# rampasek/DrVAE

Hardware: AMD Instinct MI355X
Metric: DrVAE ELBO training samples/sec (batch x L) (higher is better)
Workload: dtype f32; 1 GPU; cfg2: DrVAE bortezomib shape: 978 genes, z1=z3=100, enc-z1 800, dec-x 600, enc-z3/dec-z1 200, batch 150/GPU, L=2; global_batch=150, L=2, parallelism=dp1, launch=hipGraph replay, feed=resident, side_chain_cus=64, rccl_ranks=0, params=2321758

## Files before the change

drvae_amd/_lib.py:

```python
import ctypes as C
import os

_HERE = os.path.dirname(os.path.abspath(__file__))
LIB_PATH = os.path.join(_HERE, 'libdrvae_hip.so')

ACT = {'identity': 0, 'elu': 1, 'softplus': 2, 'sigmoid': 3, 'tanh': 4, 'relu': 5, 'leaky_relu': 6, 'selu': 7,
       'softsign': 8, 'cos': 9}
GAUSS_LOGVAR, GAUSS_SIGMA = 0, 1
REC_KIND = {'binary': 0, 'poisson': 1}
EPI_PLAIN, EPI_FWD, EPI_BWD, EPI_KLQ = 0, 1, 2, 3

_f, _i32, _i64, _u64, _p = C.c_float, C.c_int32, C.c_int64, C.c_uint64, C.c_void_p


class GemmDesc(C.Structure):
    _fields_ = [('M', _i32), ('N', _i32), ('K', _i32), ('a_kcontig', _i32), ('b_kcontig', _i32),
                ('A', _p), ('lda', _i64), ('A2', _p), ('lda2', _i64), ('K1', _i32), ('a_kscale', _p),
                ('B', _p), ('ldb', _i64), ('C', _p), ('ldc', _i64), ('alpha', _f), ('beta', _f),
                ('epilogue', _i32), ('scale', _p), ('bias', _p), ('split', _i32), ('act0', _i32), ('act1', _i32),
                ('shift0', _f), ('shift1', _f), ('resid', _p), ('ldr', _i64), ('resid_cols', _i32),
                ('yref', _p), ('ldy', _i64), ('a_colsum', _p), ('colsum_beta', _f), ('flags', _i32),
                ('pub_flag', _p), ('pub_ctr', _p), ('pub_add', _i32), ('tune', _p)]


# ... 98 lines not shown
                ('n_entries', _i32), ('max_rows', _i32), ('S', _i32), ('B', _i32), ('grp_ptr', _p), ('rows', _p), ('src', _p),
                ('cls', _p), ('W', _p), ('b', _p), ('a', _f), ('c', _f), ('w', _f), ('fac', _f), ('theta', _p), ('diff', _p),
                ('cnt', _p), ('m2', _p), ('value', _p), ('dz', _p), ('ldd', _i64)]


class LossTerm(C.Structure):
    _fields_ = [('x', _p), ('w', _p), ('n', _i32), ('scale', _f), ('out', _i32), ('row_len', _i32)]


SIGNATURES = {
    'dv_abi_version': [],
    'dv_error_string': [_i32],
    'dv_source_hash': [],
    'dv_gemm': [C.POINTER(GemmDesc), _p],
    'dv_gemm_pair': [C.POINTER(GemmDesc), C.POINTER(GemmDesc), _p],
    'dv_gemm_heads': [C.POINTER(GemmDesc), C.POINTER(HeadsEpi), _p],
    'dv_gemm_heads_tiles': [_i32],
    'dv_bn_fwd': [_p, _i64, _i32, _i32, _p, _p, _f, _p, _p, _p, _i64, _p, _p, _f, _i32, _p],
    'dv_bn_bwd': [_p, _i64, _p, _i64, _p, _p, _p, _i32, _i32, _p, _i64, _p, _p, _i32, _p],
    'dv_mask_scale': [_p, _i64, _p, _i64, _f, _i32, _i32, _p, _i64, _p],
    'dv_gemm_has_tiling': [_i32],
    'dv_colsum': [_p, _i64, _i32, _i32, _p, _f, _p],
    'dv_act_bwd': [_p, _i64, _p, _i64, _i32, _i32, _i32, _i32, _i32, _f, _f, _p],
    'dv_wn_scale': [_p, _i64, _p, _i32, _i32, _p, _p, _p],
    'dv_wn_bwd': [_p, _i64, _p, _i64, _p, _p, _i32, _i32, _p, _i64, _p, _f, _p],
    'dv_reparam_fwd': [_p, _p, _i64, _p, _i32, _i32, _i32, _p, _i64, _i32, _p, _i64, _p, _i64, _p, _i64, _p, _i64, _p,
                       _p],
    'dv_reparam_bwd_seg': [_p, _i64, _p, _i64, _p, _i64, _p, _p, _i32, _i32, _i32, _p, _i64, _p, _p, _p, _p, _i64, _f,
                           C.POINTER(Bump), C.POINTER(SegAdd), C.POINTER(Wait), C.POINTER(PriorKl), _p],
    'dv_z2f_post_bwd': [C.POINTER(Z2F), C.POINTER(Wait), _p],
    'dv_reparam_bwd': [_p, _i64, _p, _i64, _p, _i64, _p, _i32, _i32, _i32, _i32, _p, _p, _i64, _f, _p],
    'dv_kl_rows_fwd': [C.POINTER(KlRows), C.POINTER(Wait), _p],
    'dv_kl_rows_fwd_pair': [C.POINTER(KlRows), C.POINTER(KlRows), _p],
    'dv_kl_rows_bwd': [C.POINTER(KlRows), C.POINTER(KlRowsGrad), _p],
    'dv_gauss_nll_rows_fwd': [_p, _i64, _p, _p, _p, _i64, _i32, _i32, _i32, _p, _p, _p, _f, _p],
    'dv_gauss_nll_rows_fwdbwd': [_p, _p, _i64, _p, _p, _p, _i64, _i32, _i32, _i32, _i32, _f, _p, _p, _p, _i64, _p, _p, _p],
    'dv_gauss_nll_rows_raw_cs': [C.POINTER(NllRawCs), _p],
    'dv_nll_raw_cs_chunks': [_i32],
    'dv_nll_raw_cs_row_blocks': [_i32],
    'dv_rec_nll_rows': [_i32, _f, _p, _p, _i64, _p, _p, _i64, _i32, _i32, _p, _p, _i64, _p],
    'dv_gauss_nll_rows_bwd': [_p, _p, _i64, _p, _p, _p, _i64, _i32, _i32, _i32, _i32, _f, _p, _p, _i64, _p, _i64,
                              _f, _p],
    'dv_softmax_clamp_fwd': [_p, _i64, _i32, _i32, _i32, _p, _i64, _p],
    'dv_softmax_clamp_bwd': [_p, _i64, _p, _i64, _i32, _i32, _i32, _p, _i64, _f, _p],
    'dv_cat_terms_fwd': [_p, _i64, _i32, _i32, _p, _p, _i64, _p, _p, _i64, _p, _p, _p],
    'dv_cat_terms_bwd': [_p, _i64, _i32, _i32, _p, _p, _i64, _p, _p, _i64, _p, _p, _i64, _f, _p],
    'dv_smalln_linear_fwd': [_p, _i64, _i32, _p, _i64, _i32, _p, _i64, _p, _i32, _i32, _p, _i64, _p, _i64,
                             C.POINTER(Ymarg), _p, _p, _p],
    'dv_smalln_linear_bwd_data': [_p, _i64, _p, _i64, _p, _i64, _i32, _i32, _i32, C.POINTER(_p), C.POINTER(_i64),
                                  C.POINTER(_i32), C.POINTER(_i32), C.POINTER(_f), C.POINTER(_f), C.POINTER(_i32),
                                  C.POINTER(_f), _p, _i64, _p, _p],
    'dv_smalln_linear_bwd_weight': [_p, _i64, _p, _i64, _p, _i64, _i32, _p, _i64, _i32, _i32, _i32, _p, _i64, _p, _f,
                                    _p, _p, _i32, _p],
    'dv_ymarg_fwd': [_p, _i64, _p, _p, _p, _f, _p, _i32, _i32, _p, _p, _p],
    'dv_ymarg_fwdbwd': [_p, _i64, _p, _p, _p, _f, _p, _p, _p, _i32, _i32, _p, _p, _p, _p, _i64, _p],
    'dv_ymarg_bwd': [_p, _i64, _p, _p, _p, _f, _p, _p, _p, _i32, _i32, _p, _p, _i64, _p],
    'dv_ycont_fwd': [_p, _i64, _p, _p, _p, _i64, _f, _i32, _i32, _i32, _i32, _p, _p, _i64, _p, _i64, _p],
    'dv_ycont_bwd': [_p, _i64, _p, _p, _f, _i32, _p, _p, _p, _i64, _p, _i64, _i32, _i32, _i32, _p, _i64, _p, _p],
    'dv_mmd_rff_fwd': [_p, _i64, _i32, _p, _i64, _i32, _i32, _f, _p, _p, _p],
    'dv_mmd_rff_bwd': [_p, _i64, _i32, _i32, _p, _p, _f, _p, _i64, _p],
    'dv_nuisance_feed': [_p, _p, _i32, _p, _p, _i32, _p, _i32, _i32, _i32, _p, _i64, _p, _i64, _p, _p],
    'dv_mmd_grouped_fwd': [C.POINTER(MmdGrouped), _p],
    'dv_mmd_grouped_bwd': [C.POINTER(MmdGrouped), _p],
    'dv_rows_gather': [_p, _i64, _p, _i32, _i32, _p, _i64, _f, _p, _i32, _p, _i64, C.POINTER(Wait), _p],
    'dv_batch_feed': [C.POINTER(BatchFeed), C.POINTER(BatchMasks), C.POINTER(Wait), _p],
    'dv_batch_masks': [C.POINTER(BatchMasks), _p, _i32, _p, _p, _i32, _i32, _p],
    'dv_rows_segment_sum': [_p, _i64, _p, _p, _p, _i32, _i32, _p, _p, _i64, _f, C.POINTER(Wait), _p],
    'dv_weighted_sum': [_p, _p, _p, _i32, _f, _p, _f, _p],
    'dv_recon_row_stats': [_p, _i64, _p, _i64, _i32, _i32, _p, _p],
    'dv_recon_rows': [C.POINTER(ReconRows), _p],
    'dv_col_moments': [_p, _i64, _p, _i64, _i32, _i32, _p, _i32, _p, _p, _p],
    'dv_mmd_mix_fwd': [_p, _i64, _i32, _i32, _i32, _p, _i32, _p, _i64, _p, _i64, _p, _p],
    'dv_mmd_mix_bwd': [_p, _i64, _i32, _i32, _i32, _p, _i32, _p, _i64, _p, _i64, _p, _f, _p, _i64, _p, _p],
    'dv_mmd_mix_combine': [_p, _i32, _f, _p, _i32, _f, _p, _i32, _f, _p, _p],
    'dv_mmd_identity_fwd': [_p, _i64, _i32, _p, _i64, _i32, _i32, _p, _p, _p],
    'dv_mmd_identity_bwd': [_p, _p, _f, _i32, _i32, _p, _i64, _p],
    'dv_recon_finalize': [_p, _p, _i32, _i32, _p, _i32, _p, _p, _p],
    'dv_rank_metrics': [_p, _i64, _p, _p, _p, _i32, _i32, _i32, _i32, _p, _p, _p],
    'dv_loss_assemble': [C.POINTER(LossTerm), _i32, _p, _p, _p, _p, _i32, _p, _p],
    'dv_loss_assemble_after': [C.POINTER(Wait), C.POINTER(LossTerm), _i32, _p, _p, _p, C.POINTER(Bump), _p, _i32, _p, _p],
    'dv_axpby': [_p, _f, _p, _f, _i64, _p],
    'dv_adam_l2': [_p, _p, _p, _p, _i64, C.POINTER(AdamHyper), _p, _p, _i32, _p],
    'dv_adam_l2_gated': [_p, _p, _p, _p, _i64, C.POINTER(AdamHyper), _p, C.POINTER(Wait), _i64, _i64, _p, _i32, _p],
    'dv_adamax_l2': [_p, _p, _p, _p, _i64, C.POINTER(AdamHyper), _p, _p, _i32, _p],
    'dv_flag_publish': [_p, _p, _i32, _p],
    'dv_flag_wait': [_p, _p, _i32, _p, _i32, C.POINTER(Publish), _p],
    'dv_counter_add': [_p, _i32, _i64, _p],
    'dv_counters_add2': [_p, _i32, _i64, _p, _i32, _i64, _p, _p],
    'dv_fill_normal': [_p, _i64, _u64, _p, _p],
    'dv_fill_normal_rows': [_p, _p, _i32, _u64, _p, _p, _p],
}

_lib = None
ABI_VERSION = 12


def load():
    global _lib
    if _lib is not None:
        return _lib
    import torch
    path = os.environ.get('DRVAE_HIP_LIB', LIB_PATH)
    if not os.path.exists(path):
        raise RuntimeError(
            'drvae_amd: %s is missing -- build it with `python -m drvae_amd.build` (hipcc, gfx950). '
            'There is no CPU/PyTorch fallback for the hot path.' % LIB_PATH)
    lib = C.CDLL(path)
    for name, argtypes in SIGNATURES.items():
        try:
            fn = getattr(lib, name)
        except AttributeError as e:
            raise RuntimeError('drvae_amd: symbol %s missing from %s (stale build?)' % (name, LIB_PATH)) from e
        fn.argtypes = argtypes
        fn.restype = C.c_char_p if name in ('dv_error_string', 'dv_source_hash') else C.c_int
    if lib.dv_abi_version() != ABI_VERSION:
        raise RuntimeError('drvae_amd: ABI version mismatch in %s' % LIB_PATH)
    _lib = lib
    return lib


def check(code, what):
    if code != 0:
        msg = load().dv_error_string(code)
        raise RuntimeError('drvae_amd: %s failed: %s (%d)' % (what, msg.decode() if msg else '?', code))
```

drvae_amd/chain.py:

```python
import torch

from . import kernels as K


def _pad4(n):
    return (n + 3) // 4 * 4


def _whole_rows(t):
    b = t._base
    return (b is not None and b.dim() == 2 and t.dim() == 2 and b.is_contiguous() and t.stride() == (b.shape[1], 1)
            and b.shape[1] == _pad4(t.shape[1]) and (t.storage_offset() - b.storage_offset()) % b.shape[1] == 0)


class _Lin:

    def __init__(self, arena, wname, bname, gname=None, second=None, act='identity', act1=None, shift0=0.0,
                 shift1=0.0):
        if second is None:
            self.W, self.dW = arena.p(wname), arena.g(wname)
            self.b, self.db = arena.p(bname), arena.g(bname)
            self.g = arena.p(gname) if gname else None
            self.dg = arena.g(gname) if gname else None
            self.split = self.W.shape[0]
        else:
            w2, b2, g2 = second
            self.W, self.dW = arena.fused(arena.param, wname, w2), arena.fused(arena.grad, wname, w2)
            self.b, self.db = arena.fused(arena.param, bname, b2), arena.fused(arena.grad, bname, b2)
            self.g = arena.fused(arena.param, gname, g2) if gname and g2 else None
            self.dg = arena.fused(arena.grad, gname, g2) if gname and g2 else None
            self.split = arena.shapes[wname][0]
        self.N, self.Kin = self.W.shape
        self.act0, self.act1 = act, (act if act1 is None else act1)
        self.shift0, self.shift1 = shift0, shift1
        dev = self.W.device
        if self.g is not None:
            self.scale = torch.empty(self.N, device=dev)
            self.norm = torch.empty(self.N, device=dev)
            self.raw = torch.empty(self.N, self.Kin, device=dev)
        else:
            self.scale = self.norm = self.raw = None


class _Chain:

    def __init__(self, layers, M, device, resid_cols=0):
        self.layers, self.M, self.resid_cols = layers, M, resid_cols
        self.out = [torch.zeros(M, _pad4(l.N), device=device)[:, :l.N] for l in layers]
        self.dpre = [torch.zeros(M, _pad4(l.N), device=device)[:, :l.N] for l in layers[:-1]]

    @staticmethod
    def _pad_ok(t):
        if t.dim() != 2 or t.shape[1] % 4 == 0:
            return True
        ld = t.stride(0) if t.shape[0] > 1 else max(t.stride(0), t.shape[1])
        return ld == t.shape[1] or _whole_rows(t)

    def raw_last_ok(self):
        l = self.layers[-1]
        return l.g is None and l.split * 2 == l.N and l.act0 == 'identity' and self.resid_cols == 0

    def forward(self, inputs, resid=None, publish=None, heads=None, raw_last=False):
        x = list(inputs)
        for li, l in enumerate(self.layers):
            if l.g is not None:
                K.wn_scale(l.scale, l.norm, l.W, l.g)
            last = li == len(self.layers) - 1
            kpad = len(x) == 1 and self._pad_ok(x[0])
            if last and heads is not None:
                assert l.split * 2 == l.N
                K.linear_heads(heads.get('out', self.out[li]), x[0], l.W, l.b, split=l.split,
                               x2=x[1] if len(x) > 1 else None, scale=l.scale, act0=l.act0, act1=l.act1,
                               shift0=l.shift0, shift1=l.shift1, resid=resid,
                               resid_cols=self.resid_cols if resid is not None else 0, overread=True,
                               publish=publish if (li == 0 and l.g is None) else None,
                               sample=heads.get('sample'), nll=heads.get('nll'), kpad=kpad)
                return self.out[-1]
            if last and raw_last:
                assert self.raw_last_ok() and resid is None
                K.gemm(self.out[li], x[0], l.W, True, True, A2=x[1] if len(x) > 1 else None, overread=True,
                       publish=publish if li == 0 else None, kpad=kpad)
                return self.out[-1]
            K.linear_fwd(self.out[li], x[0], l.W, l.b, x2=x[1] if len(x) > 1 else None, scale=l.scale, split=l.split,
                         act0=l.act0, act1=l.act1, shift0=l.shift0, shift1=l.shift1,
                         resid=resid if last else None, resid_cols=self.resid_cols if (last and resid is not None) else 0,
                         overread=True, publish=publish if (li == 0 and l.g is None) else None, kpad=kpad)
            x = [self.out[li]]
        return self.out[-1]

    def backward(self, dpre_last, inputs, dinputs=None, publish_after_last=None, publish_first=None, db_last_done=False,
                 klq=None):
        dpre = dpre_last
        pending_pub = publish_first
        took_klq = False
        n_layers = len(self.layers)
        for li in range(n_layers - 1, -1, -1):
            l = self.layers[li]
            db = None if (db_last_done and li == n_layers - 1) else l.db
            srcs = list(inputs) if li == 0 else [self.out[li - 1]]
            if li == len(self.layers) - 2 and publish_after_last is not None:
                pending_pub = publish_after_last

            single_dst = li > 0 or (dinputs is not None and len(srcs) == 1 and dinputs[0] is not None
                                    and len(dinputs[0]) == 1)
            if l.g is None and len(srcs) == 1 and single_dst:
                if li > 0:
                    prev = self.layers[li - 1]
                    K.linear_bwd_pair(l.dW, db, self.dpre[li - 1], dpre, srcs[0], l.W, yref=self.out[li - 1],
                                      act=prev.act0, shift=prev.shift0, overread=True, publish=pending_pub,
                                      npad=self._pad_ok(srcs[0]), npad_x=True)
                    dpre = self.dpre[li - 1]
                else:
                    dst, alpha, beta = dinputs[0][0]
                    if klq is not None and beta == 0.0:
                        K.linear_bwd_pair(l.dW, db, None, dpre, srcs[0], l.W, alpha=alpha, overread=True, publish=pending_pub,
                                          npad=self._pad_ok(srcs[0]), klq=klq)
                        took_klq = True
                    else:
                        K.linear_bwd_pair(l.dW, db, dst, dpre, srcs[0], l.W, alpha=alpha, beta_x=beta, overread=True,
                                          publish=pending_pub, npad=self._pad_ok(srcs[0]), npad_x=_whole_rows(dst))
                pending_pub = None
                continue
            if pending_pub is not None:
                K.flag_publish(*pending_pub)
                pending_pub = None
            dW = l.raw if l.g is not None else l.dW
            c0 = 0
            for si, s in enumerate(srcs):
                w = s.shape[1]
                K.linear_bwd_weight(dW[:, c0:c0 + w], dpre, s, dbias=db if si == 0 else None, overread=True,
                                    npad=len(srcs) == 1 and l.g is None and self._pad_ok(s))
                c0 += w
            if l.g is not None:
                K.wn_bwd(l.dW, l.dg, l.raw, l.W, l.g, l.norm)
            if li > 0:
                prev = self.layers[li - 1]
                K.linear_bwd_data(self.dpre[li - 1], dpre, l.W, kscale=l.scale, yref=self.out[li - 1], act=prev.act0,
                                  shift=prev.shift0, overread=True, npad=True)
                dpre = self.dpre[li - 1]
            elif dinputs is not None:
                c0 = 0
                for si, s in enumerate(srcs):
                    w = s.shape[1]
                    for (dst, alpha, beta) in (dinputs[si] or []):
                        K.linear_bwd_data(dst, dpre, l.W[:, c0:c0 + w], kscale=l.scale, alpha=alpha, beta=beta,
                                          overread=True)
                    c0 += w
        return took_klq
```

drvae_amd/csrc/gemm.hip:

```cpp
#include "gemm_common.inc"

namespace {

#include "gemm_pipe.inc"


struct Operand {
    const float* base;
    int64_t ld;
    int n_line, n_pos;
};

__device__ __forceinline__ float4 ld_fast(const Operand& o, int line, int pos, int vec) {
    const float* p = o.base + (int64_t)line * o.ld + pos;
    if (vec == 4) return *reinterpret_cast<const float4*>(p);
    if (vec == 2) {
        const float2 a = *reinterpret_cast<const float2*>(p), b = *reinterpret_cast<const float2*>(p + 2);
        return make_float4(a.x, a.y, b.x, b.y);
    }
    return make_float4(p[0], p[1], p[2], p[3]);
}

__device__ __forceinline__ float4 ld_edge(const Operand& o, int line, int pos) {
    const bool lok = line < o.n_line;
    const float* row = o.base + (int64_t)(lok ? line : o.n_line - 1) * o.ld;
    float e[4];
#pragma unroll
    for (int j = 0; j < 4; ++j) {
        const int q = pos + j;
        const float v = row[q < o.n_pos ? q : o.n_pos - 1];
        e[j] = (lok && q < o.n_pos) ? v : 0.f;
    }
    return make_float4(e[0], e[1], e[2], e[3]);
}

template <int BM, int RPT>
__device__ __forceinline__ int heads_row0(int grp) { return (grp & 1) * (BM / 2) + (grp >> 1) * RPT; }

template <int BM, int BN, int KS, int NT>
__device__ __forceinline__ void heads_epilogue(const dv_gemm_desc& g, const dv_heads_epi& he, const float* red, int m0,
                                               int tn, int tiles_n, int pre_s0, int pre_s1) {
    constexpr int HB = BN / 2, RPT = BM / (NT / HB);
    constexpr bool PRE = (KS == 8 && BN == 32);
    static_assert(!PRE || RPT == 1, "prefetched bounds: one row per thread");
    static_assert((HB == 32 || HB == 16) && RPT >= 1, "half tile = 16 or 32 adjacent lanes");
    static_assert((NT / HB) % 2 == 0 && (BM / 2) % RPT == 0, "row groups come in pairs");
    const int tid = threadIdx.x, c = tid % HB, r0 = heads_row0<BM, RPT>(tid / HB);
    const int col0 = tn * HB + c, col1 = g.split + col0;
    const bool ok = col0 < g.split && col1 < g.N;
    const int cc0 = ok ? col0 : g.split - 1, cc1 = ok ? col1 : g.N - 1;
    float sc0 = 1.f, sc1 = 1.f, bi0 = 0.f, bi1 = 0.f;
    if (g.scale) {
        sc0 = g.scale[cc0];
        sc1 = g.scale[cc1];
    }
    if (g.bias) {
        bi0 = g.bias[cc0];
        bi1 = g.bias[cc1];
    }
    const bool use_res = g.resid != nullptr && col0 < g.resid_cols;
#pragma unroll
    for (int e = 0; e < RPT; ++e) {
        const int row = m0 + r0 + e;
        const bool rok = row < g.M;
        const int rc = rok ? row : g.M - 1;
        float v0 = 0.f, v1 = 0.f;
#pragma unroll
        for (int w = 0; w < KS; ++w) {
            v0 += red[(w * BM + r0 + e) * (BN + 1) + c];
            v1 += red[(w * BM + r0 + e) * (BN + 1) + HB + c];
        }
        float a0 = dv_act(g.act0, v0 * g.alpha * sc0 + bi0) + g.shift0;
        if (use_res) a0 += g.resid[(int64_t)rc * g.ldr + cc0];
        if (he.mode == DV_HEADS_NLL && g.act1 == DV_ACT_SOFTPLUS) {
            const float pre = v1 * g.alpha * sc1 + bi1;
            const float e_ = __expf(-fabsf(pre));
            const float r1 = __frcp_rn(1.f + e_);
            const float sd = fmaxf(pre, 0.f) + dv_log1p_hw(e_, r1) + g.shift1;
            const float sig = (pre >= 0.f ? 1.f : e_) * r1;
            const float is = __frcp_rn(sd);
            const float xv = he.x[(int64_t)(he.xidx ? he.xidx[rc] : rc) * he.ldx + cc0];
            const float cf = he.coef[rc];
            const float t = (xv - a0) * is;
            float acc = ok ? kLog2PiG + 2.f * __logf(sd) + t * t : 0.f;
            if (ok && rok) {
                g.C[(int64_t)row * g.ldc + col0] = cf * t * is;
                g.C[(int64_t)row * g.ldc + col1] = cf * (t * t - 1.f) * is * sig;
            }
#pragma unroll
            for (int off = HB / 2; off > 0; off >>= 1) acc += __shfl_xor(acc, off, 64);
            if (c == 0 && rok) he.part[(int64_t)row * tiles_n + tn] = -0.5f * acc;
            continue;
        }
        const float a1 = dv_act(g.act1, v1 * g.alpha * sc1 + bi1) + g.shift1;
        if (he.mode == DV_HEADS_SAMPLE) {
            if (ok && rok) {
                g.C[(int64_t)row * g.ldc + col0] = a0;
                g.C[(int64_t)row * g.ldc + col1] = a1;
                if (row < he.n_src) {
                    const float std_ = expf(0.5f * a1);
                    const int s0 = he.seg_ptr ? (PRE ? pre_s0 : he.seg_ptr[row]) : row;
                    const int s1 = he.seg_ptr ? (PRE ? pre_s1 : he.seg_ptr[row + 1]) : row + 1;
                    for (int t = s0; t < s1; ++t) {
                        const int64_t s = he.seg_rows ? he.seg_rows[t] : t;
                        const float z = he.eps[s * he.lde + col0] * std_ + a0;
                        he.out[s * he.ldo + col0] = z;
                        if (he.out2) he.out2[s * he.ldo2 + col0] = z - he.sub[s * he.lds + col0];
                        if (he.out3) {
                            const int t3 = he.out3_idx[s];
                            if (t3 >= 0) he.out3[(int64_t)t3 * he.ldo3 + col0] = z;
                        }
                        if (he.out4)
                            for (int u = he.out4_ptr[s]; u < he.out4_ptr[s + 1]; ++u) he.out4[(int64_t)u * he.ldo4 + col0] = z;
                    }
                }
            }
        } else {
            const float xv = he.x[(int64_t)(he.xidx ? he.xidx[rc] : rc) * he.ldx + cc0];
            const float cf = he.coef[rc];
            const float d = xv - a0, v = a1 * a1;
            float acc = ok ? kLog2PiG + logf(v) + d * d / v : 0.f;
            float gm = d / v, gs = -1.f / a1 + d * d / (v * a1);
            if (g.act1 != DV_ACT_IDENTITY) gs *= dv_dact_from_y(g.act1, a1 - g.shift1);
            gm *= cf;
            gs *= cf;
            if (ok && rok) {
                g.C[(int64_t)row * g.ldc + col0] = gm;
                g.C[(int64_t)row * g.ldc + col1] = gs;
            }
#pragma unroll
            for (int off = HB / 2; off > 0; off >>= 1) acc += __shfl_xor(acc, off, 64);
            if (c == 0 && rok) he.part[(int64_t)row * tiles_n + tn] = -0.5f * acc;
        }
    }
}

template <int BM, int BN, int BK, int KS, bool AKC, bool BKC, int PS = 0>
constexpr int gemm_smem_floats() {
    if constexpr (PS > 0) return PipeGeom<BM, BN, BK, BM / 32, BN / 32, KS, PS, AKC, BKC>::SMEM_FL;
    constexpr int stage = (AKC ? BM : BK) * ((AKC ? BK : BM) + 4) + (BKC ? BN : BK) * ((BKC ? BK : BN) + 4);
    constexpr int red = (KS > 1) ? KS * BM * (BN + 1) : 0;
    return 2 * stage > red ? 2 * stage : red;
}

template <int BM, int BN, int BK, int WM, int WN, int KS, bool AKC, bool BKC, bool PAIR = false, bool MI16 = false, int PS = 0>
__device__ __forceinline__ void gemm_body(const dv_gemm_desc& g, const LoadCfg& lc, float* smem, int bid, int nwg,
                                          const dv_heads_epi* he = nullptr) {
    static_assert(!PAIR || (AKC && BKC && KS > 1 && WM == 1 && WN == 1), "paired heads: forward layout, K-split tiling");
    constexpr int HB = BN / 2;
    static_assert(!MI16 || (KS == 1 && !PAIR), "16x16x4 tiles: unsplit K only");
    constexpr int TS = MI16 ? 16 : 32;
    constexpr int AR = MI16 ? 4 : 16;
    constexpr int TM = BM / WM / TS, TN = BN / WN / TS;
    constexpr int KW = BK / KS, KH = KW / (MI16 ? 4 : 2);
    constexpr int LDA_S = (AKC ? BK : BM) + 4;
    constexpr int LDB_S = (BKC ? BK : BN) + 4;
    constexpr int A_ELEMS = (AKC ? BM : BK) * LDA_S;
    constexpr int B_ELEMS = (BKC ? BN : BK) * LDB_S;
    constexpr int STAGE = A_ELEMS + B_ELEMS;
    constexpr int RED_ELEMS = (KS > 1) ? KS * BM * (BN + 1) : 0;
    constexpr int NT = 64 * WM * WN * KS;
    static_assert(PS > 0 || (2 * STAGE <= gemm_smem_floats<BM, BN, BK, KS, AKC, BKC>() && RED_ELEMS <= gemm_smem_floats<BM, BN, BK, KS, AKC, BKC>()), "smem");
    static_assert(PS == 0 || (!MI16 && TM == 1 && TN == 1), "pipe loop inside gemm_body: one 32x32 tile per wave");
    static_assert(NT == 256 || NT == 512 || NT == 1024, "4, 8 or 16 waves");

    const bool ones_col = BM < 128 && !AKC && !BKC && (g.flags & DV_FLAG_ONES_COL);
    const int tiles_m = (g.M + BM - 1) / BM;
    const int tiles_n = PAIR ? (g.split + HB - 1) / HB : (g.N + (ones_col ? DV_ONES_OFF(g) + 1 : 0) + BN - 1) / BN;
    int tm, tn;
    tile_of_block(bid, nwg, tiles_m, tiles_n, lc.map, tm, tn);
    const int m0 = tm * BM, n0 = tn * BN;
    auto bline = [&](int l) -> int {
        if (PAIR) {
            const int c = tn * HB + (l < HB ? l : l - HB);
            return l < HB ? (c < g.split ? c : g.split - 1) : (g.split + c < g.N ? g.split + c : g.N - 1);
        }
        return n0 + l < g.N ? n0 + l : g.N - 1;
    };

    const int tid = threadIdx.x, lane = tid & 63, wave = tid >> 6;
    const int li = MI16 ? (lane & 15) : (lane & 31), lh = MI16 ? (lane >> 4) : (lane >> 5);
    const int ks_id = wave / (WM * WN);
    const int wm = (wave % (WM * WN)) / WN, wn = wave % WN;

    constexpr int A_CPL = (AKC ? BK : BM) / 4;
    constexpr int A_LPP = NT / A_CPL;
    constexpr int A_NP = (AKC ? BM : BK) / A_LPP;
    constexpr int B_CPL = (BKC ? BK : BN) / 4;
    constexpr int B_LPP = NT / B_CPL;
    constexpr int B_NP = (BKC ? BN : BK) / B_LPP;
    static_assert(A_NP >= 1 && B_NP >= 1, "tile too small for the workgroup");
    const int a_c = tid % A_CPL, a_l = tid / A_CPL;
    const int b_c = tid % B_CPL, b_l = tid / B_CPL;
    const int oc = (ones_col && n0 <= g.N && g.N < n0 + BN) ? g.N - n0 - b_c * 4 : -1;

    const Operand oa{g.A, g.lda, AKC ? g.M : g.K, AKC ? g.K : g.M};
    const Operand ob{g.B, g.ldb, BKC ? g.N : g.K, BKC ? g.K : g.N};
    const bool a_plain = g.A2 == nullptr;
    const bool a_int = AKC ? true : (m0 + BM <= g.M);
    const bool b_int = BKC ? true : (n0 + BN <= g.N);
    const bool wg_fast = a_plain && (a_int || (g.flags & 1)) && (b_int || (g.flags & 2)) && g.a_kscale == nullptr;

    auto gen_load = [&](int k0, float4 (&ra)[A_NP], float4 (&rb)[B_NP]) {
#pragma unroll
        for (int p = 0; p < A_NP; ++p) {
            const int l = a_l + p * A_LPP;
            const int line = AKC ? (m0 + l) : (k0 + l);
            const int pos = AKC ? (k0 + a_c * 4) : (m0 + a_c * 4);
            float4 v;
            if (a_plain) {
                v = ld_edge(oa, line, pos);
            } else {
                const bool lok = line < g.M;
                const int64_t r = lok ? line : g.M - 1;
                float e[4];
#pragma unroll
                for (int j = 0; j < 4; ++j) {
                    const int q = pos + j, qc = q < g.K ? q : g.K - 1;
                    const float* src = qc >= g.K1 ? g.A2 + r * g.lda2 + (qc - g.K1) : g.A + r * g.lda + qc;
                    const float x = *src;
                    e[j] = (lok && q < g.K) ? x : 0.f;
                }
                v = make_float4(e[0], e[1], e[2], e[3]);
            }
            if (AKC && g.a_kscale) {
                const int kq = g.K - 1;
                v.x *= g.a_kscale[pos < kq ? pos : kq];
                v.y *= g.a_kscale[pos + 1 < kq ? pos + 1 : kq];
                v.z *= g.a_kscale[pos + 2 < kq ? pos + 2 : kq];
                v.w *= g.a_kscale[pos + 3 < kq ? pos + 3 : kq];
// ... 26 lines not shown
        }
    };

    typename std::conditional<MI16, f32x4, f32x16>::type acc[TM][TN];
#pragma unroll
    for (int i = 0; i < TM; ++i)
#pragma unroll
        for (int j = 0; j < TN; ++j)
#pragma unroll
            for (int r = 0; r < AR; ++r) acc[i][j][r] = 0.f;

    int pre_s0 = 0, pre_s1 = 0;
    if constexpr (PAIR && KS == 8 && BN == 32) {
        if (he->mode == DV_HEADS_SAMPLE && he->seg_ptr != nullptr) {
            const int prow = m0 + heads_row0<BM, 1>(tid / (BN / 2));
            if (prow < he->n_src && prow < g.M) {
                pre_s0 = he->seg_ptr[prow];
                pre_s1 = he->seg_ptr[prow + 1];
            }
        }
    }
    const int kb = ks_id * KW + lh * KH;
    auto read_frags = [&](const float* sA, float (&fa)[TM][KH], float (&fb)[TN][KH]) {
        const float* sB = sA + A_ELEMS;
#pragma unroll
        for (int i = 0; i < TM; ++i) {
            const int row = wm * TM * TS + i * TS + li;
#pragma unroll
            for (int s = 0; s < KH; s += 4) {
                if (AKC) {
                    const float4 v = *reinterpret_cast<const float4*>(&sA[row * LDA_S + kb + s]);
                    fa[i][s] = v.x;
                    fa[i][s + 1] = v.y;
                    fa[i][s + 2] = v.z;
                    fa[i][s + 3] = v.w;
                } else {
#pragma unroll
                    for (int e = 0; e < 4; ++e) fa[i][s + e] = sA[(kb + s + e) * LDA_S + row];
                }
            }
        }
#pragma unroll
        for (int j = 0; j < TN; ++j) {
            const int col = wn * TN * TS + j * TS + li;
#pragma unroll
            for (int s = 0; s < KH; s += 4) {
                if (BKC) {
                    const float4 v = *reinterpret_cast<const float4*>(&sB[col * LDB_S + kb + s]);
                    fb[j][s] = v.x;
                    fb[j][s + 1] = v.y;
                    fb[j][s + 2] = v.z;
                    fb[j][s + 3] = v.w;
                } else {
#pragma unroll
                    for (int e = 0; e < 4; ++e) fb[j][s + e] = sB[(kb + s + e) * LDB_S + col];
                }
            }
        }
    };
    auto mma = [&](const float (&fa)[TM][KH], const float (&fb)[TN][KH]) {
#pragma unroll
        for (int s = 0; s < KH; ++s)
#pragma unroll
            for (int i = 0; i < TM; ++i)
#pragma unroll
                for (int j = 0; j < TN; ++j) {
                    if constexpr (MI16)
                        acc[i][j] = __builtin_amdgcn_mfma_f32_16x16x4f32(fa[i][s], fb[j][s], acc[i][j], 0, 0, 0);
                    else if (DV_DBG & 2)
                        acc[i][j][s & 15] += fa[i][s] * fb[j][s];
                    else
                        acc[i][j] = __builtin_amdgcn_mfma_f32_32x32x2f32(fa[i][s], fb[j][s], acc[i][j], 0, 0, 0);
                }
    };
    auto compute = [&](const float* sA) {
        float fa[TM][KH], fb[TN][KH];
        read_frags(sA, fa, fb);
        mma(fa, fb);
    };

    const int nkt = (g.K + BK - 1) / BK, nfull = g.K / BK;
    float* const buf0 = smem;
    float* const buf1 = smem + STAGE;
    if constexpr (PS > 0) {
        if (!(DV_DBG & 64))
            pipe_loop<BM, BN, BK, WM, WN, KS, PS, AKC, BKC, (BM < 128 && !AKC && !BKC)>(
                g, smem, m0, n0, [&](int l) { return m0 + l < g.M ? m0 + l : g.M - 1; }, bline, acc);
        if (DV_DBG & 128) {
            if (acc[0][0][0] == 12345.678f) g.C[0] = acc[0][0][1];
            return;
        }
        __syncthreads();
    } else if (wg_fast && nfull >= 1) {
        const float* pa[A_NP];
        const float* pb[B_NP];
#pragma unroll
        for (int p = 0; p < A_NP; ++p) {
            const int l = a_l + p * A_LPP;
            int line = AKC ? (m0 + l) : l;
            if (AKC) line = line < g.M ? line : g.M - 1;
            pa[p] = g.A + (int64_t)line * g.lda + (AKC ? a_c * 4 : (m0 + a_c * 4 < g.M ? m0 + a_c * 4 : 0));
        }
#pragma unroll
        for (int p = 0; p < B_NP; ++p) {
            const int l = b_l + p * B_LPP;
            const int line = BKC ? bline(l) : l;
            pb[p] = g.B + (int64_t)line * g.ldb + (BKC ? b_c * 4 : (n0 + b_c * 4 < g.N ? n0 + b_c * 4 : 0));
        }
        const int64_t step_a = AKC ? (int64_t)BK : (int64_t)BK * g.lda;
        const int64_t step_b = BKC ? (int64_t)BK : (int64_t)BK * g.ldb;
        const int va = lc.vecA, vb = lc.vecB;
        auto ldv = [](const float* p, int vec) -> float4 {
            if (vec == 4) return *reinterpret_cast<const float4*>(p);
            if (vec == 2) {
                const float2 a = *reinterpret_cast<const float2*>(p), b = *reinterpret_cast<const float2*>(p + 2);
                return make_float4(a.x, a.y, b.x, b.y);
            }
            return make_float4(p[0], p[1], p[2], p[3]);
        };
        auto ldv_tail = [](const float* p, int vec, int left) -> float4 {
            const float* z = dv_zero_chunk;
            if (vec == 4) return *reinterpret_cast<const float4*>(left >= 4 ? p : z);
            if (vec == 2) {
                const float2 a = *reinterpret_cast<const float2*>(left >= 2 ? p : z);
                const float2 b = *reinterpret_cast<const float2*>(left >= 4 ? p + 2 : z);
                return make_float4(a.x, a.y, b.x, b.y);
            }
            return make_float4(*(left >= 1 ? p : z), *(left >= 2 ? p + 1 : z), *(left >= 3 ? p + 2 : z),
                               *(left >= 4 ? p + 3 : z));
        };
        auto fetch = [&](int t, float4 (&ra)[A_NP], float4 (&rb)[B_NP]) {
            if (t < nfull) {
#pragma unroll
                for (int p = 0; p < A_NP; ++p) {
                    ra[p] = ldv(pa[p], va);
                    pa[p] += step_a;
                }
#pragma unroll
                for (int p = 0; p < B_NP; ++p) {
                    rb[p] = ldv(pb[p], vb);
                    pb[p] += step_b;
                }
            } else {
                const int kt0 = nfull * BK;
#pragma unroll
                for (int p = 0; p < A_NP; ++p) {
                    if (AKC) {
                        ra[p] = ldv_tail(pa[p], lc.vecA_t, g.K - (kt0 + a_c * 4));
                    } else {
                        ra[p] = ldv((kt0 + a_l + p * A_LPP < g.K) ? pa[p] : dv_zero_chunk, va);
                    }
                }
#pragma unroll
                for (int p = 0; p < B_NP; ++p) {
                    if (BKC) {
                        rb[p] = ldv_tail(pb[p], lc.vecB_t, g.K - (kt0 + b_c * 4));
                    } else {
                        rb[p] = ldv((kt0 + b_l + p * B_LPP < g.K) ? pb[p] : dv_zero_chunk, vb);
                    }
                }
            }
        };
        float4 a0[A_NP], b0[B_NP], a1[A_NP], b1[B_NP];
#if DV_STAMP
        const bool stamp_on = dv_stamp_buf != nullptr && wave == 0;
        int si = 2;
#endif
// ... 49 lines not shown
            }
            if (!(DV_DBG & 8)) __syncthreads();
            if (kt + 1 >= nkt) break;
            compute(buf1);
            if (kt + 2 < nkt) {
                if (!(DV_DBG & 4)) stage_store(buf0, a0, b0);
                if (kt + 4 < nkt && !(DV_DBG & 1)) fetch(kt + 4, a0, b0);
            }
            if (!(DV_DBG & 8)) __syncthreads();
        }
    } else {
        float4 ra[A_NP], rb[B_NP];
        gen_load(0, ra, rb);
        stage_store(buf0, ra, rb);
        __syncthreads();
        for (int kt = 0; kt < nkt; ++kt) {
            if (kt + 1 < nkt) gen_load((kt + 1) * BK, ra, rb);
            compute((kt & 1) ? buf1 : buf0);
            if (kt + 1 < nkt) stage_store((kt & 1) ? buf0 : buf1, ra, rb);
            __syncthreads();
        }
    }

    if constexpr (MI16) {
#pragma unroll
        for (int i = 0; i < TM; ++i)
#pragma unroll
            for (int j = 0; j < TN; ++j) {
                float a4[4];
#pragma unroll
                for (int r = 0; r < 4; ++r) a4[r] = acc[i][j][r];
                const int rbase = m0 + wm * TM * TS + i * TS + 4 * lh;
                epi_store_col<4, (BM < 128)>(g, a4, n0 + wn * TN * TS + j * TS + li, [rbase](int r) { return rbase + r; });
            }
    } else if constexpr (KS == 1) {
#pragma unroll
        for (int i = 0; i < TM; ++i)
#pragma unroll
            for (int j = 0; j < TN; ++j) {
                float a16[16];
#pragma unroll
                for (int r = 0; r < 16; ++r) a16[r] = acc[i][j][r];
                const int rbase = m0 + wm * TM * 32 + i * 32 + 4 * lh;
                epi_store_col<16, (BM < 128)>(g, a16, n0 + wn * TN * 32 + j * 32 + li,
                                  [rbase](int r) { return rbase + (r & 3) + 8 * (r >> 2); });
            }
    } else {
        float* red = smem;
        if constexpr (PAIR) {
#pragma unroll
            for (int j = 0; j < TN; ++j)
#pragma unroll
                for (int r = 0; r < 16; ++r) {
                    const int row = (r & 3) + 8 * (r >> 2) + 4 * lh;
                    red[(ks_id * BM + row) * (BN + 1) + j * 32 + li] = acc[0][j][r];
                }
            __syncthreads();
            heads_epilogue<BM, BN, KS, NT>(g, *he, red, m0, tn, tiles_n, pre_s0, pre_s1);
            return;
        }
#pragma unroll
        for (int i = 0; i < TM; ++i)
#pragma unroll
            for (int j = 0; j < TN; ++j)
#pragma unroll
                for (int r = 0; r < 16; ++r) {
                    const int row = wm * TM * 32 + i * 32 + (r & 3) + 8 * (r >> 2) + 4 * lh;
                    const int col = wn * TN * 32 + j * 32 + li;
                    red[(ks_id * BM + row) * (BN + 1) + col] = acc[i][j][r];
                }
        __syncthreads();
        constexpr int RPT = BM / (NT / BN);
        const int col = tid % BN, r0 = (tid / BN) * RPT;
        float a4[RPT];
#pragma unroll
        for (int e = 0; e < RPT; ++e) {
            float v = 0.f;
#pragma unroll
            for (int w = 0; w < KS; ++w) v += red[(w * BM + r0 + e) * (BN + 1) + col];
            a4[e] = v;
        }
        const int rbase = m0 + r0;
        epi_store_col<RPT>(g, a4, n0 + col, [rbase](int r) { return rbase + r; });
    }
}


template <int BM, int BN, int BK, int WM, int WN, int KS, bool AKC, bool BKC, bool MI16 = false>
__global__ __launch_bounds__(64 * WM * WN * KS, (WM * WN * KS == 16) ? 4 : (BM >= 128 || BK >= 128) ? 2 : (BM * BN >= 6144) ? (WM * WN * KS) / 4 : (WM * WN * KS == 8 ? (BM * BN == 1024 ? DV_LB8 : 2) : (BK == 32 && BM == 32 ? ((AKC || BKC) ? DV_DENSE_WG : DV_DENSE_WG - 1) : 4))) void gemm_kernel(const dv_gemm_desc g, const LoadCfg lc) {
    __shared__ __attribute__((aligned(16))) float smem[gemm_smem_floats<BM, BN, BK, KS, AKC, BKC>()];
    publish_on_entry(g);
#if DV_STAGGER
    {
        const int ph = (blockIdx.x / DV_STAGGER) & 3;
        if (ph == 1) __builtin_amdgcn_s_sleep(6);
        if (ph == 2) __builtin_amdgcn_s_sleep(12);
        if (ph == 3) __builtin_amdgcn_s_sleep(18);
    }
#endif
    gemm_body<BM, BN, BK, WM, WN, KS, AKC, BKC, false, MI16>(g, lc, smem, blockIdx.x, gridDim.x);
}

#ifdef DV_LAB
template <int KS, int NBUF = 3>
__global__ __launch_bounds__(64 * KS, NBUF > 4 ? KS / 4 : (KS == 8 ? 2 : 4)) void gemm_dma_kernel(const dv_gemm_desc g, const LoadCfg lc) {
    constexpr int BM = 32, BN = 32, BK = 64, NT = 64 * KS, KW = BK / KS, KH = KW / 2;
    constexpr int TILE = 32 * BK, STAGE = 2 * TILE, RED = KS * BM * (BN + 1);
    constexpr int PIECES = 16 / KS;
    static_assert((NBUF - 2) * PIECES <= 63, "vmcnt is a 6-bit counter");
    __shared__ __attribute__((aligned(16))) float smem[NBUF * STAGE > RED ? NBUF * STAGE : RED];
    publish_on_entry(g);
    const int tiles_m = (g.M + BM - 1) / BM, tiles_n = (g.N + BN - 1) / BN;
    int tm, tn;
    tile_of_block(blockIdx.x, gridDim.x, tiles_m, tiles_n, lc.map, tm, tn);
    const int m0 = tm * BM, n0 = tn * BN;
    const int tid = threadIdx.x, lane = tid & 63, wave = tid >> 6;
    const int li = lane & 31, lh = lane >> 5;

    const float* src[PIECES];
    int kofs[PIECES];
    int dst[PIECES];
#pragma unroll
    for (int i = 0; i < PIECES; ++i) {
        const int q = wave + i * KS, o = q >> 3, row = 4 * (q & 7) + (lane >> 4), p = lane & 15;
        const int c = p ^ (row & 15);
        int line = (o == 0 ? m0 : n0) + row;
        const int lim = o == 0 ? g.M : g.N;
        line = line < lim ? line : lim - 1;
        src[i] = (o == 0 ? g.A + (int64_t)line * g.lda : g.B + (int64_t)line * g.ldb) + c * 4;
        kofs[i] = c * 4;
        dst[i] = o * TILE + (q & 7) * 256;
    }
    auto issue = [&](int kt, float* stage) {
#pragma unroll
        for (int i = 0; i < PIECES; ++i) {
            const float* p = (kt * BK + kofs[i] < g.K) ? src[i] + (int64_t)kt * BK : dv_zero_chunk;
            __builtin_amdgcn_global_load_lds(p, (__attribute__((address_space(3))) float*)(stage + dst[i]), 16, 0, 0);
        }
    };
    f32x16 acc;
#pragma unroll
    for (int r = 0; r < 16; ++r) acc[r] = 0.f;
    const int kb = wave * KW + lh * KH;
    const int nkt = (g.K + BK - 1) / BK;
#pragma unroll
    for (int t = 0; t < NBUF - 1; ++t) issue(t, smem + t * STAGE);
    int bi = 0;
    for (int kt = 0; kt < nkt; ++kt) {
        float* cur = smem + bi * STAGE;
        asm volatile("s_waitcnt vmcnt(%0)" ::"n"((NBUF - 2) * PIECES) : "memory");
        asm volatile("s_barrier" ::: "memory");
        int bn = bi + NBUF - 1;
        bn = bn >= NBUF ? bn - NBUF : bn;
        issue(kt + NBUF - 1, smem + bn * STAGE);
        bi = bi + 1 == NBUF ? 0 : bi + 1;
        float fa[KH], fb[KH];
#pragma unroll
        for (int s = 0; s < KH; s += 4) {
            const int pc = (((kb + s) >> 2) ^ (li & 15)) << 2;
            const float4 va = *reinterpret_cast<const float4*>(&cur[li * BK + pc]);
            const float4 vb = *reinterpret_cast<const float4*>(&cur[TILE + li * BK + pc]);
            fa[s] = va.x; fa[s + 1] = va.y; fa[s + 2] = va.z; fa[s + 3] = va.w;
            fb[s] = vb.x; fb[s + 1] = vb.y; fb[s + 2] = vb.z; fb[s + 3] = vb.w;
        }
#pragma unroll
        for (int s = 0; s < KH; ++s) acc = __builtin_amdgcn_mfma_f32_32x32x2f32(fa[s], fb[s], acc, 0, 0, 0);
// ... 70 lines not shown
        const float4 x0 = *reinterpret_cast<const float4*>(&(ST)[li * LD + lh * 8]);       \
        const float4 x1 = *reinterpret_cast<const float4*>(&(ST)[li * LD + lh * 8 + 4]);   \
        const float4 y0 = *reinterpret_cast<const float4*>(&(ST)[OPER + li * LD + lh * 8]);     \
        const float4 y1 = *reinterpret_cast<const float4*>(&(ST)[OPER + li * LD + lh * 8 + 4]); \
        acc = __builtin_amdgcn_mfma_f32_32x32x2f32(x0.x, y0.x, acc, 0, 0, 0);              \
        acc = __builtin_amdgcn_mfma_f32_32x32x2f32(x0.y, y0.y, acc, 0, 0, 0);              \
        acc = __builtin_amdgcn_mfma_f32_32x32x2f32(x0.z, y0.z, acc, 0, 0, 0);              \
        acc = __builtin_amdgcn_mfma_f32_32x32x2f32(x0.w, y0.w, acc, 0, 0, 0);              \
        acc = __builtin_amdgcn_mfma_f32_32x32x2f32(x1.x, y1.x, acc, 0, 0, 0);              \
        acc = __builtin_amdgcn_mfma_f32_32x32x2f32(x1.y, y1.y, acc, 0, 0, 0);              \
        acc = __builtin_amdgcn_mfma_f32_32x32x2f32(x1.z, y1.z, acc, 0, 0, 0);              \
        acc = __builtin_amdgcn_mfma_f32_32x32x2f32(x1.w, y1.w, acc, 0, 0, 0);              \
    }
    if (s0 < s1) {
        float* st0 = my;
        float* st1 = my + STAGE;
        WP_FETCH(s0, a00, a01, b00, b01);
        WP_FETCH(s0 + 1, a10, a11, b10, b11);
        WP_STASH(st0, a00, a01, b00, b01);
        WP_FETCH(s0 + 2, a00, a01, b00, b01);
        const int n = s1 - s0;
        int s = s0;
        for (int it = 0; it < n / 2; ++it, s += 2) {
            WP_STASH(st1, a10, a11, b10, b11);
            WP_FETCH(s + 3, a10, a11, b10, b11);
            WP_MMA(st0);
            WP_STASH(st0, a00, a01, b00, b01);
            WP_FETCH(s + 4, a00, a01, b00, b01);
            WP_MMA(st1);
        }
        if (n & 1) WP_MMA(st0);
    }
#undef WP_FETCH
#undef WP_STASH
#undef WP_MMA
    __syncthreads();
    float* red = smem;
#pragma unroll
    for (int r = 0; r < 16; ++r) red[(wave * BM + (r & 3) + 8 * (r >> 2) + 4 * lh) * (BN + 1) + li] = acc[r];
    __syncthreads();
    constexpr int RPT = BM / (256 / BN);
    const int col = tid % BN, r0 = (tid / BN) * RPT;
    float a4[RPT];
#pragma unroll
    for (int e = 0; e < RPT; ++e) {
        float v = 0.f;
#pragma unroll
        for (int w = 0; w < KS; ++w) v += red[(w * BM + r0 + e) * (BN + 1) + col];
        a4[e] = v;
    }
    const int rbase = m0 + r0;
    epi_store_col<RPT>(g, a4, n0 + col, [rbase](int r) { return rbase + r; });
}

#endif

template <int BM, int BN, int BK, int KS>
__global__ __launch_bounds__(64 * KS, KS == 8 ? 2 : (BK == 32 ? DV_DENSE_WG : 4)) void gemm_heads_kernel(const dv_gemm_desc g, const LoadCfg lc,
                                                               const dv_heads_epi he) {
    __shared__ __attribute__((aligned(16))) float smem[gemm_smem_floats<BM, BN, BK, KS, true, true>()];
    publish_on_entry(g);
    gemm_body<BM, BN, BK, 1, 1, KS, true, true, true>(g, lc, smem, blockIdx.x, gridDim.x, &he);
}

template <int BM, int BN, int BK, int WM, int WN, int KS, bool A1, bool B1, bool A2, bool B2>
__global__ __launch_bounds__(256, BK == 32 ? DV_DENSE_WG : 4) void gemm_pair_kernel(const dv_gemm_desc g1, const LoadCfg lc1, const dv_gemm_desc g2,
                                                        const LoadCfg lc2, int tiles1) {
    constexpr int S1 = gemm_smem_floats<BM, BN, BK, KS, A1, B1>(), S2 = gemm_smem_floats<BM, BN, BK, KS, A2, B2>();
    __shared__ __attribute__((aligned(16))) float smem[S1 > S2 ? S1 : S2];
    publish_on_entry(g1);
    if ((int)blockIdx.x < tiles1)
        gemm_body<BM, BN, BK, WM, WN, KS, A1, B1>(g1, lc1, smem, blockIdx.x, tiles1);
    else
        gemm_body<BM, BN, BK, WM, WN, KS, A2, B2>(g2, lc2, smem, blockIdx.x - tiles1, gridDim.x - tiles1);
}

template <int BM, int BN, int BK, int KS, bool AKC, bool BKC, int PS, int WPS>
__global__ __launch_bounds__(64 * KS * (BM / 32) * (BN / 32), WPS) void gemm_kpipe_kernel(const dv_gemm_desc g, const LoadCfg lc) {
    __shared__ __attribute__((aligned(1024))) float smem[gemm_smem_floats<BM, BN, BK, KS, AKC, BKC, PS>()];
    publish_on_entry(g);
    gemm_body<BM, BN, BK, BM / 32, BN / 32, KS, AKC, BKC, false, false, PS>(g, lc, smem, blockIdx.x, gridDim.x);
}

template <int BM, int BN, int BK, int KS, int PS, int WPS>
__global__ __launch_bounds__(64 * KS, WPS) void gemm_heads_pipe_kernel(const dv_gemm_desc g, const LoadCfg lc, const dv_heads_epi he) {
    __shared__ __attribute__((aligned(1024))) float smem[gemm_smem_floats<BM, BN, BK, KS, true, true, PS>()];
    publish_on_entry(g);
    gemm_body<BM, BN, BK, 1, 1, KS, true, true, true, false, PS>(g, lc, smem, blockIdx.x, gridDim.x, &he);
}

template <int BM, int BN, int BK, int KS, bool A1, bool B1, bool A2, bool B2, int PS, int WPS>
__global__ __launch_bounds__(256, WPS) void gemm_pair_pipe_kernel(const dv_gemm_desc g1, const LoadCfg lc1, const dv_gemm_desc g2,
                                                                    const LoadCfg lc2, int tiles1) {
    constexpr int S1 = gemm_smem_floats<BM, BN, BK, KS, A1, B1, PS>(), S2 = gemm_smem_floats<BM, BN, BK, KS, A2, B2, PS>();
    __shared__ __attribute__((aligned(1024))) float smem[S1 > S2 ? S1 : S2];
    publish_on_entry(g1);
    if ((int)blockIdx.x < tiles1)
        gemm_body<BM, BN, BK, 1, 1, KS, A1, B1, false, false, PS>(g1, lc1, smem, blockIdx.x, tiles1);
    else
        gemm_body<BM, BN, BK, 1, 1, KS, A2, B2, false, false, PS>(g2, lc2, smem, blockIdx.x - tiles1, gridDim.x - tiles1);
}

inline int vec_width(const void* p, int64_t ld) {
    const uintptr_t a = reinterpret_cast<uintptr_t>(p);
    if ((a & 15) == 0 && (ld & 3) == 0) return 4;
    if ((a & 7) == 0 && (ld & 1) == 0) return 2;
    return 1;
}

const dv_gemm_tune k_default_tune = {0, {-1, 0, 0, 0, 0, 0, 0, 0, 0, 0}};
inline const dv_gemm_tune& tune_of(const dv_gemm_desc& g) { return g.tune != nullptr ? *g.tune : k_default_tune; }
inline int lds_pad(const dv_gemm_desc& g, int bm, int tiles) { return (bm <= 32 && tiles >= 512) ? tune_of(g).opt[1] : 0; }

inline int cols_eff(const dv_gemm_desc& g) { return g.N + ((g.flags & DV_FLAG_ONES_COL) ? DV_ONES_OFF(g) + 1 : 0); }

template <int BM, int BN, int BK, int WM, int WN, int KS, bool MI16 = false>
int launch_cfg(const dv_gemm_desc& g, const LoadCfg& lc, hipStream_t st) {
    const int tiles = ((g.M + BM - 1) / BM) * ((cols_eff(g) + BN - 1) / BN);
    dim3 grid(tiles), block(64 * WM * WN * KS);
    if (g.a_kcontig && g.b_kcontig)
        hipLaunchKernelGGL((gemm_kernel<BM, BN, BK, WM, WN, KS, true, true, MI16>), grid, block, lds_pad(g, BM, tiles), st, g, lc);
    else if (g.a_kcontig && !g.b_kcontig)
        hipLaunchKernelGGL((gemm_kernel<BM, BN, BK, WM, WN, KS, true, false, MI16>), grid, block, lds_pad(g, BM, tiles), st, g, lc);
    else if (!g.a_kcontig && !g.b_kcontig)
        hipLaunchKernelGGL((gemm_kernel<BM, BN, BK, WM, WN, KS, false, false, MI16>), grid, block, lds_pad(g, BM, tiles), st, g, lc);
    else
        return DV_ERR_UNSUPPORTED;
    DV_RETURN_LAUNCH();
}

inline void pipe_ones_off(dv_gemm_desc& g) {
    if (g.flags & DV_FLAG_ONES_COL) g.flags = (g.flags & ~0x300) | (((4 - (g.N & 3)) & 3) << 8);
}

template <int BM, int BN, int BK, int KS, int PS, int WPS>
int launch_kpipe(const dv_gemm_desc& g_in, const LoadCfg& lc, hipStream_t st) {
    dv_gemm_desc g = g_in;
    pipe_ones_off(g);
    const int tiles = ((g.M + BM - 1) / BM) * ((cols_eff(g) + BN - 1) / BN);
    dim3 grid(tiles), block(64 * KS * (BM / 32) * (BN / 32));
    if (g.a_kcontig && g.b_kcontig)
        hipLaunchKernelGGL((gemm_kpipe_kernel<BM, BN, BK, KS, true, true, PS, WPS>), grid, block, 0, st, g, lc);
    else if (g.a_kcontig && !g.b_kcontig)
        hipLaunchKernelGGL((gemm_kpipe_kernel<BM, BN, BK, KS, true, false, PS, WPS>), grid, block, 0, st, g, lc);
    else if (!g.a_kcontig && !g.b_kcontig)
        hipLaunchKernelGGL((gemm_kpipe_kernel<BM, BN, BK, KS, false, false, PS, WPS>), grid, block, 0, st, g, lc);
    else
        return DV_ERR_UNSUPPORTED;
    DV_RETURN_LAUNCH();
}

}

extern "C" int dv_gemm_has_tiling(int t) {
#ifndef DV_LAB
    return ((t >= 0 && t <= 3) || t == 17 || t == 40 || t == 46) ? 1 : 0;
#else
    return t >= 0 ? 1 : 0;
#endif
}

#if DV_STAMP
extern "C" int dv_gemm_stamp_buffer(unsigned long long* p) {
    return hipMemcpyToSymbol(HIP_SYMBOL(dv_stamp_buf), &p, sizeof(p)) == hipSuccess ? DV_OK : DV_ERR_LAUNCH;
}
#endif
// ... 114 lines not shown
            DV_RETURN_LAUNCH();
        }
        return launch_cfg<32, 32, 64, 1, 1, 8>(g, lc, st);
    }
    if (tiling == 11 || tiling == 12 || (tiling >= 21 && tiling <= 24)) {
        const bool ok = g.a_kcontig && g.b_kcontig && g.A2 == nullptr && g.a_kscale == nullptr && (g.K & 3) == 0 &&
                        lc.vecA == 4 && lc.vecB == 4;
        if (ok) {
            const int tiles = ((g.M + 31) / 32) * ((g.N + 31) / 32);
            if (tiling == 11)
                hipLaunchKernelGGL((gemm_dma_kernel<8>), dim3(tiles), dim3(512), 0, st, g, lc);
            else if (tiling == 12)
                hipLaunchKernelGGL((gemm_dma_kernel<4>), dim3(tiles), dim3(256), 0, st, g, lc);
            else if (tiling == 21)
                hipLaunchKernelGGL((gemm_dma_kernel<8, 5>), dim3(tiles), dim3(512), 0, st, g, lc);
            else if (tiling == 22)
                hipLaunchKernelGGL((gemm_dma_kernel<8, 9>), dim3(tiles), dim3(512), 0, st, g, lc);
            else if (tiling == 23)
                hipLaunchKernelGGL((gemm_dma_kernel<4, 5>), dim3(tiles), dim3(256), 0, st, g, lc);
            else
                hipLaunchKernelGGL((gemm_dma_kernel<4, 9>), dim3(tiles), dim3(256), 0, st, g, lc);
            DV_RETURN_LAUNCH();
        }
        return launch_cfg<32, 32, 64, 1, 1, 8>(g, lc, st);
    }
#endif
    if (tiling == 17) return launch_cfg<32, 32, 32, 1, 1, 4>(g, lc, st);
    if (tiling != 1 && tiling != 2) return DV_ERR_UNSUPPORTED;
    if (tiling == 1) return launch_cfg<64, 64, 32, 2, 2, 1>(g, lc, st);
    const int tiles32 = ((g.M + 31) / 32) * ((cols_eff(g) + 31) / 32);
    const bool pipe = pipe_on(g) && pipe_ok(g, lc);
    if (tiles32 >= dense_min_tiles(g)) return pipe ? launch_kpipe<32, 32, 32, 4, 2, DV_DENSE_WG>(g, lc, st) : launch_cfg<32, 32, 32, 1, 1, 4>(g, lc, st);
    if (g.a_kcontig && tune_of(g).opt[7] == 0) return pipe ? launch_kpipe<32, 32, 64, 8, 2, 2>(g, lc, st) : launch_cfg<32, 32, 64, 1, 1, 8>(g, lc, st);
    return pipe ? launch_kpipe<32, 32, 64, 4, 2, 4>(g, lc, st) : launch_cfg<32, 32, 64, 1, 1, 4>(g, lc, st);
}

static bool ragged_n_split_pays(const dv_gemm_desc& g, int tiling) {
    if (tiling != 40 || tune_of(g).tiling != 0 || tune_of(g).opt[6] == -1) return false;
    const int n_tail = g.N % 256, n_main = g.N - n_tail;
    if (n_tail == 0 || n_main == 0) return false;
    const int64_t rows_t = (g.M + 127) / 128, kCUs = 256;
    const int64_t full = rows_t * ((g.N + 255) / 256), main = rows_t * (n_main / 256);
    return (full + kCUs - 1) / kCUs > (main + kCUs - 1) / kCUs;
}

extern "C" int dv_gemm(const dv_gemm_desc* d, dv_stream_t stream) {
    LoadCfg lc;
    int tiling = 0;
    const int rc = gemm_prepare(d, lc, tiling);
    if (rc != DV_OK) return rc;
    if (ragged_n_split_pays(*d, tiling)) {
        const int n_tail = d->N % 256, n_main = d->N - n_tail;
        dv_gemm_desc g1 = *d, g2 = *d;
        g1.N = n_main;
        g2.N = n_tail;
        g2.B = d->B + (d->b_kcontig ? (int64_t)n_main * d->ldb : (int64_t)n_main);
        g2.C = d->C + n_main;
        g1.split = d->split < n_main ? d->split : n_main;
        g2.split = d->split > n_main ? d->split - n_main : 0;
        if (d->scale) g2.scale = d->scale + n_main;
        if (d->bias) g2.bias = d->bias + n_main;
        if (d->yref) g2.yref = d->yref + n_main;
        if (d->resid) {
            g1.resid_cols = d->resid_cols < n_main ? d->resid_cols : n_main;
            g2.resid_cols = d->resid_cols > n_main ? d->resid_cols - n_main : 0;
            g2.resid = g2.resid_cols > 0 ? d->resid + n_main : nullptr;
        }
        g2.a_colsum = nullptr;
        g2.pub_flag = nullptr;
        g2.tune = nullptr;
        LoadCfg l1, l2;
        int t1 = 0, t2 = 0;
        int r = gemm_prepare(&g1, l1, t1);
        if (r != DV_OK) return r;
        r = gemm_prepare(&g2, l2, t2);
        if (r != DV_OK) return r;
        r = gemm_launch(g1, l1, t1, static_cast<hipStream_t>(stream));
        if (r != DV_OK) return r;
        return gemm_launch(g2, l2, t2, static_cast<hipStream_t>(stream));
    }
    return gemm_launch(*d, lc, tiling, static_cast<hipStream_t>(stream));
}

#ifdef DV_LAB
static int heads_hb() { return 16; }
#else
static int heads_hb() { return 16; }
#endif
extern "C" int dv_gemm_heads_tiles(int32_t split) { return split > 0 ? (split + heads_hb() - 1) / heads_hb() : 0; }

extern "C" int dv_gemm_heads(const dv_gemm_desc* d, const dv_heads_epi* e, dv_stream_t stream) {
    LoadCfg lc;
    int tiling = 0;
    DV_REQUIRE(d != nullptr && e != nullptr);
    const int rc = gemm_prepare(d, lc, tiling);
    if (rc != DV_OK) return rc;
    if (tiling < 0) return DV_OK;
    const dv_gemm_desc& g = *d;
    DV_REQUIRE(g.a_kcontig && g.b_kcontig && g.epilogue == DV_EPI_FWD && g.beta == 0.f && g.a_colsum == nullptr);
    DV_REQUIRE(g.split > 0 && g.N == 2 * g.split && g.resid_cols <= g.split);
    DV_REQUIRE(e->mode == DV_HEADS_SAMPLE || e->mode == DV_HEADS_NLL);
    if (e->mode == DV_HEADS_SAMPLE) {
        DV_REQUIRE(e->eps && e->out && e->n_src >= 0 && e->n_src <= g.M);
        DV_REQUIRE((e->seg_ptr == nullptr) == (e->seg_rows == nullptr));
        DV_REQUIRE(e->out2 == nullptr || e->sub != nullptr);
        DV_REQUIRE(e->out3 == nullptr || e->out3_idx != nullptr);
        DV_REQUIRE(e->out4 == nullptr || e->out4_ptr != nullptr);
    } else {
        DV_REQUIRE(e->x && e->coef && e->part);
    }
    lc.map = tune_of(g).opt[0] >= 0 ? tune_of(g).opt[0] : 1;
    const int tiles = ((g.M + 31) / 32) * dv_gemm_heads_tiles(g.split);
#ifdef DV_LAB
    if (tune_of(g).opt[4] == 1) {
        hipLaunchKernelGGL((gemm_heads_kernel<32, 64, 64, 4>), dim3(tiles), dim3(256), 0,
                           static_cast<hipStream_t>(stream), g, lc, *e);
        DV_RETURN_LAUNCH();
    }
    if (tune_of(g).opt[4] == 2) {
        hipLaunchKernelGGL((gemm_heads_kernel<32, 64, 64, 8>), dim3(tiles), dim3(512), 0,
                           static_cast<hipStream_t>(stream), g, lc, *e);
        DV_RETURN_LAUNCH();
    }
    if (tune_of(g).opt[4] == -1) {
        hipLaunchKernelGGL((gemm_heads_kernel<32, 32, 64, 4>), dim3(tiles), dim3(256), 0,
                           static_cast<hipStream_t>(stream), g, lc, *e);
        DV_RETURN_LAUNCH();
    }
#endif
    const bool pipe = pipe_on(g) && pipe_ok(g, lc);
    if (tune_of(g).opt[4] == 3 || (tune_of(g).opt[4] == 0 && tiles >= dense_min_tiles(g))) {
        if (pipe)
            hipLaunchKernelGGL((gemm_heads_pipe_kernel<32, 32, 32, 4, 2, DV_DENSE_WG>), dim3(tiles), dim3(256), 0,
                               static_cast<hipStream_t>(stream), g, lc, *e);
        else
            hipLaunchKernelGGL((gemm_heads_kernel<32, 32, 32, 4>), dim3(tiles), dim3(256), 0,
                               static_cast<hipStream_t>(stream), g, lc, *e);
    } else if (pipe) {
        hipLaunchKernelGGL((gemm_heads_pipe_kernel<32, 32, 64, 8, 2, 2>), dim3(tiles), dim3(512), 0,
                           static_cast<hipStream_t>(stream), g, lc, *e);
    } else {
        hipLaunchKernelGGL((gemm_heads_kernel<32, 32, 64, 8>), dim3(tiles), dim3(512), lds_pad(g, 32, tiles),
                           static_cast<hipStream_t>(stream), g, lc, *e);
    }
    DV_RETURN_LAUNCH();
}

extern "C" int dv_gemm_pair(const dv_gemm_desc* d1, const dv_gemm_desc* d2, dv_stream_t stream) {
    LoadCfg lc1, lc2;
    int t1 = 0, t2 = 0;
    int rc = gemm_prepare(d1, lc1, t1);
    if (rc != DV_OK) return rc;
    rc = gemm_prepare(d2, lc2, t2);
    if (rc != DV_OK) return rc;
    hipStream_t st = static_cast<hipStream_t>(stream);
    DV_REQUIRE(!(d1->pub_flag != nullptr && d2->pub_flag != nullptr));
    dv_gemm_desc e1 = *d1, e2 = *d2;
    e2.flags &= 3;
    if (t1 == 2 && t2 == 2) {
        rc = colsum_setup(e1, 2, st);
        if (rc != DV_OK) return rc;
    }
    const bool pipe = pipe_on(e1) && t1 == 2 && t2 == 2 && pipe_ok(e1, lc1) && pipe_ok(e2, lc2);
    if (pipe) pipe_ones_off(e1);
    const int tiles1 = ((e1.M + 31) / 32) * ((cols_eff(e1) + 31) / 32), tiles2 = ((e2.M + 31) / 32) * ((e2.N + 31) / 32);
    const bool fuse = t1 == 2 && t2 == 2 && !d1->a_kcontig && !d1->b_kcontig && d2->a_kcontig && !d2->b_kcontig &&
// ... 38 lines not shown
```

drvae_amd/csrc/gemm_pipe.inc:

```

template <int BM, int BN, int BK, int WM, int WN, int KS, int S, bool AKC, bool BKC>
struct PipeGeom {
    static constexpr int NW = WM * WN * KS, NT = 64 * NW;
    static constexpr int TM = BM / WM / 32, TN = BN / WN / 32;
    static constexpr int KW = BK / KS, KH = KW / 2, G = KH / 4;
    static constexpr int A_FL = BM * BK, B_FL = BN * BK, STAGE_FL = A_FL + B_FL;
    static constexpr int PA = A_FL / 256, PB = B_FL / 256, P = (PA + PB) / NW;
    static constexpr int CPR = BK / 4;
    static constexpr int RED_FL = (KS > 1) ? KS * BM * (BN + 1) : 0;
    static constexpr int SMEM_FL = S * STAGE_FL > RED_FL ? S * STAGE_FL : RED_FL;
    static_assert(KH % 4 == 0 && G >= 1, "a lane half holds whole 16-B chunks of k");
    static_assert((PA + PB) % NW == 0 && P >= 1, "pieces divide over the waves");
    static_assert(CPR == 4 || CPR == 8 || CPR == 16, "BK = 16, 32 or 64");
    static_assert(TM == 1 || TM == 2 || TM == 4, "row-contiguous reads are 4, 8 or 16 B");
    static_assert(TN == 1 || TN == 2 || TN == 4, "row-contiguous reads are 4, 8 or 16 B");
    static_assert(AKC || (256 % BM == 0 && BM <= 256), "row-contiguous A: whole k lines per piece");
    static_assert(BKC || (256 % BN == 0 && BN <= 256), "row-contiguous B: whole k lines per piece");
    static_assert((S - 2) * P <= 63 && S >= 2, "vmcnt is a 6-bit counter");
};

template <int CPR>
__device__ __forceinline__ int pipe_sw(int row) {
    return (row / (16 / CPR)) & (CPR - 1);
}

template <int N>
__device__ __forceinline__ void pipe_wait_vm() {
    asm volatile("s_waitcnt vmcnt(%0)" ::"n"(N) : "memory");
}

template <int BM, int BN, int BK, int WM, int WN, int KS, int S, bool AKC, bool BKC, bool ONES = false, typename LineA,
          typename LineB>
__device__ __forceinline__ void pipe_loop(const dv_gemm_desc& g, float* smem, int m0, int n0, LineA a_line,
                                          LineB b_line, f32x16 (&acc)[BM / WM / 32][BN / WN / 32]) {
    using PG = PipeGeom<BM, BN, BK, WM, WN, KS, S, AKC, BKC>;
    constexpr int TM = PG::TM, TN = PG::TN, G = PG::G, P = PG::P, CPR = PG::CPR, NW = PG::NW;
    const int tid = threadIdx.x, lane = tid & 63;
    const int wave = __builtin_amdgcn_readfirstlane(tid >> 6);
    const int li = lane & 31, lh = lane >> 5;
    const int ks_id = wave / (WM * WN), wm = (wave % (WM * WN)) / WN, wn = wave % WN;

    unsigned voff[P];
    int kofs[P];
    bool live[P];
    const bool ones_on = ONES && (g.flags & DV_FLAG_ONES_COL) != 0;
    const int n_ones = g.N + DV_ONES_OFF(g);
#pragma unroll
    for (int i = 0; i < P; ++i) {
        const int q = wave + i * NW;
        const bool isA = q < PG::PA;
        const int pq = isA ? q : q - PG::PA;
        const bool kc = isA ? AKC : BKC;
        const int64_t ld = isA ? g.lda : g.ldb;
        live[i] = true;
        if (kc) {
            const int row_t = pq * (64 / CPR) + lane / CPR;
            const int c = (lane % CPR) ^ pipe_sw<CPR>(row_t);
            const int T = isA ? TM : TN, wq = row_t / (T * 32), jq = (row_t / 32) % T, lq = row_t % 32;
            const int line = isA ? a_line(wq * T * 32 + T * lq + jq) : b_line(wq * T * 32 + T * lq + jq);
            kofs[i] = c * 4;
            voff[i] = (unsigned)(((int64_t)line * ld + c * 4) * 4);
        } else {
            const int R = isA ? BM : BN;
            const int line_t = pq * (256 / R) + lane / (R / 4), rc = lane % (R / 4);
            const int r0 = isA ? m0 : n0, lim = isA ? g.M : g.N;
            const int col = r0 + rc * 4 < lim ? r0 + rc * 4 : 0;
            kofs[i] = line_t;
            voff[i] = (unsigned)(((int64_t)line_t * ld + col) * 4);
            if (ONES && !isA) live[i] = !(ones_on && r0 + rc * 4 == n_ones);
        }
    }
    const int64_t step_a = (AKC ? (int64_t)BK : (int64_t)BK * g.lda) * 4, step_b = (BKC ? (int64_t)BK : (int64_t)BK * g.ldb) * 4;
    const char* base_a = reinterpret_cast<const char*>(g.A);
    const char* base_b = reinterpret_cast<const char*>(g.B);
    int k_issued = 0;
    const unsigned lds0 = (unsigned)(uintptr_t)smem;
    auto issue_piece = [&](auto full, int i, unsigned stage_byte) {
        const int q = wave + i * NW;
        const unsigned dst = __builtin_amdgcn_readfirstlane(lds0 + stage_byte + q * 1024);
        const char* base = q < PG::PA ? base_a : base_b;
        if (DV_DBG & 16) return;
        if constexpr (decltype(full)::value) {
            if (!ONES || live[i])
                asm volatile("s_mov_b32 m0, %1\n\ts_nop 0\n\tglobal_load_lds_dwordx4 %0, %2" ::"v"(voff[i]), "s"(dst), "s"(base) : "memory");
        } else if (!ONES || live[i]) {
            const char* p = kofs[i] < g.K - k_issued ? base + voff[i] : reinterpret_cast<const char*>(dv_zero_chunk);
            asm volatile("s_mov_b32 m0, %1\n\ts_nop 0\n\tglobal_load_lds_dwordx4 %0, off" ::"v"(p), "s"(dst) : "memory");
        }
    };
    auto issued = [&]() {
        base_a += step_a;
        base_b += step_b;
        k_issued += BK;
    };
    const int kb = ks_id * PG::KW + lh * PG::KH;
    const int swl = pipe_sw<CPR>(li);
    constexpr int NRA = AKC ? TM : 4, NRB = BKC ? TN : 4, NR = NRA + NRB;
    auto read_ops = [&](const float* stage, int gi, float (&fa)[TM][4], float (&fb)[TN][4], int lo, int hi) {
        const float* sA = stage;
        const float* sB = stage + PG::A_FL;
        const int c = ((kb >> 2) + gi) ^ swl;
#pragma unroll
        for (int r = 0; r < NRA; ++r) {
            if (r < lo || r >= hi) continue;
            if constexpr (AKC) {
                const float4 v = *reinterpret_cast<const float4*>(&sA[(wm * TM * 32 + r * 32 + li) * BK + c * 4]);
                fa[r][0] = v.x; fa[r][1] = v.y; fa[r][2] = v.z; fa[r][3] = v.w;
            } else {
                const float* p = &sA[(kb + gi * 4 + r) * BM + wm * TM * 32 + TM * li];
                if constexpr (TM == 4) {
                    const float4 v = *reinterpret_cast<const float4*>(p);
                    fa[0][r] = v.x; fa[1][r] = v.y; fa[2][r] = v.z; fa[3][r] = v.w;
                } else if constexpr (TM == 2) {
                    const float2 v = *reinterpret_cast<const float2*>(p);
                    fa[0][r] = v.x; fa[1][r] = v.y;
                } else {
                    fa[0][r] = *p;
                }
            }
        }
#pragma unroll
        for (int r = 0; r < NRB; ++r) {
            if (NRA + r < lo || NRA + r >= hi) continue;
            if constexpr (BKC) {
                const float4 v = *reinterpret_cast<const float4*>(&sB[(wn * TN * 32 + r * 32 + li) * BK + c * 4]);
                fb[r][0] = v.x; fb[r][1] = v.y; fb[r][2] = v.z; fb[r][3] = v.w;
            } else {
                const float* p = &sB[(kb + gi * 4 + r) * BN + wn * TN * 32 + TN * li];
                if constexpr (TN == 4) {
                    const float4 v = *reinterpret_cast<const float4*>(p);
                    fb[0][r] = v.x; fb[1][r] = v.y; fb[2][r] = v.z; fb[3][r] = v.w;
                } else if constexpr (TN == 2) {
                    const float2 v = *reinterpret_cast<const float2*>(p);
                    fb[0][r] = v.x; fb[1][r] = v.y;
                } else {
                    fb[0][r] = *p;
                }
            }
        }
    };
    auto read_group = [&](const float* stage, int gi, float (&fa)[TM][4], float (&fb)[TN][4]) {
        read_ops(stage, gi, fa, fb, 0, NR);
    };
    auto mma = [&](const float (&fa)[TM][4], const float (&fb)[TN][4], int lo, int hi) {
#pragma unroll
        for (int s = 0; s < 4; ++s)
#pragma unroll
            for (int i = 0; i < TM; ++i)
#pragma unroll
                for (int j = 0; j < TN; ++j) {
                    const int n = (s * TM + i) * TN + j;
                    if (n >= lo && n < hi) {
                        if (DV_DBG & 32) {
                            acc[i][j][0] += fa[i][s] + fb[j][s];
                        } else {
                            acc[i][j] = __builtin_amdgcn_mfma_f32_32x32x2f32(fa[i][s], fb[j][s], acc[i][j], 0, 0, 0);
                        }
                    }
                }
    };
    constexpr int NM = 4 * TM * TN;
    constexpr int RPM = (NR + NM - 1) / NM > 2 ? (NR + NM - 1) / NM : 2, NSL = (NR + RPM - 1) / RPM;
    static_assert(NSL <= NM, "reads dealt out over the group's MFMAs");
    const int nkt = (g.K + BK - 1) / BK;
    if constexpr (ONES) {
        if (ones_on && n0 <= n_ones && n_ones < n0 + BN && tid < S * BK)
            *reinterpret_cast<float4*>(&smem[(tid / BK) * PG::STAGE_FL + PG::A_FL + (tid % BK) * BN + (n_ones - n0)]) =
                make_float4(1.f, 1.f, 1.f, 1.f);
    }
#pragma unroll
    for (int t = 0; t < S; ++t) {
        if (k_issued + BK <= g.K) {
#pragma unroll
            for (int i = 0; i < P; ++i) issue_piece(std::true_type{}, i, t * PG::STAGE_FL * 4);
        } else {
#pragma unroll
            for (int i = 0; i < P; ++i) issue_piece(std::false_type{}, i, t * PG::STAGE_FL * 4);
        }
        issued();
    }
    asm volatile("s_waitcnt lgkmcnt(0)" ::: "memory");
    pipe_wait_vm<(S - 1) * P>();
    __builtin_amdgcn_s_barrier();
    float fa0[TM][4], fb0[TN][4], fa1[TM][4], fb1[TN][4];
    read_group(smem, 0, fa0, fb0);
    int sc = 0;
    auto tile = [&](auto full, float (&xa)[TM][4], float (&xb)[TN][4], float (&ya)[TM][4], float (&yb)[TN][4]) {
        const float* cur = smem + sc * PG::STAGE_FL;
        const int sn = sc + 1 == S ? 0 : sc + 1;
        const float* nxt = smem + sn * PG::STAGE_FL;
#pragma unroll
        for (int gi = 0; gi < G; ++gi) {
            float(&ca)[TM][4] = (gi & 1) ? ya : xa;
            float(&cb)[TN][4] = (gi & 1) ? yb : xb;
            float(&na)[TM][4] = (gi & 1) ? xa : ya;
            float(&nb)[TN][4] = (gi & 1) ? xb : yb;
            if (gi + 1 < G) {
                mma(ca, cb, 0, 1);
                __builtin_amdgcn_sched_barrier(0);
#pragma unroll
                for (int q = 0; q < NSL; ++q) {
                    read_ops(cur, gi + 1, na, nb, q * RPM, (q + 1) * RPM);
                    __builtin_amdgcn_sched_barrier(0);
                    if (q + 1 < NSL) {
                        mma(ca, cb, 1 + q, 2 + q);
                        __builtin_amdgcn_sched_barrier(0);
                    }
                }
                mma(ca, cb, NSL, NM);
                __builtin_amdgcn_sched_barrier(0);
            } else {
                asm volatile("s_waitcnt lgkmcnt(0)" ::: "memory");
                pipe_wait_vm<(S - 2) * P>();
                __builtin_amdgcn_s_barrier();
                asm volatile("" ::: "memory");
                mma(ca, cb, 0, 1);
                __builtin_amdgcn_sched_barrier(0);
#pragma unroll
                for (int q = 0; q < NSL; ++q) {
                    read_ops(nxt, 0, na, nb, q * RPM, (q + 1) * RPM);
                    __builtin_amdgcn_sched_barrier(0);
                    if (q + 1 < NSL) {
                        mma(ca, cb, 1 + q, 2 + q);
                        __builtin_amdgcn_sched_barrier(0);
                    }
                }
                const unsigned sb = sc * PG::STAGE_FL * 4;
                constexpr int M0 = NSL, ML = NM - M0;
#pragma unroll
                for (int i = 0; i < P; ++i) {
                    mma(ca, cb, M0 + i * ML / (P + 1), M0 + (i + 1) * ML / (P + 1));
                    __builtin_amdgcn_sched_barrier(0);
                    issue_piece(full, i, sb);
                    __builtin_amdgcn_sched_barrier(0);
                }
                mma(ca, cb, M0 + P * ML / (P + 1), NM);
                __builtin_amdgcn_sched_barrier(0);
                issued();
            }
        }
        sc = sn;
    };
    const int nfast = g.K / BK - S;
    int kt = 0;
    if constexpr (G % 2 == 0) {
        for (; kt < nfast; ++kt) tile(std::true_type{}, fa0, fb0, fa1, fb1);
        for (; kt < nkt; ++kt) tile(std::false_type{}, fa0, fb0, fa1, fb1);
    } else {
        for (; kt + 1 < nfast; kt += 2) {
            tile(std::true_type{}, fa0, fb0, fa1, fb1);
            tile(std::true_type{}, fa1, fb1, fa0, fb0);
        }
        for (; kt + 1 < nkt; kt += 2) {
            tile(std::false_type{}, fa0, fb0, fa1, fb1);
            tile(std::false_type{}, fa1, fb1, fa0, fb0);
        }
        if (kt < nkt) tile(std::false_type{}, fa0, fb0, fa1, fb1);
    }
    pipe_wait_vm<0>();
}

template <int BM, int BN, int WM, int WN, bool AKC, bool BKC>
__device__ __forceinline__ void pipe_epilogue(const dv_gemm_desc& g, int m0, int n0,
// ... 181 lines not shown
```

drvae_amd/csrc/optim.hip:

```cpp
#include "dv_common.h"
#include <cstring>

namespace {

struct AdamC {
    float lr_over_bc1, inv_unused, bc2_sqrt, eps, wd, one_minus_b1, b2, one_minus_b2, gscale;
};

__device__ __forceinline__ void adam_consts(float lr, float b1, float b2, const int32_t* step_dev, float* step_size,
                                            float* bc2_sqrt) {
    const double t = (double)step_dev[0];
    const double bc1 = 1.0 - pow((double)b1, t);
    const double bc2 = 1.0 - pow((double)b2, t);
    *step_size = (float)((double)lr / bc1);
    *bc2_sqrt = (float)sqrt(bc2);
}

__device__ __forceinline__ void adam_one(float& p, float g, float& m, float& v, float step_size, float bc2_sqrt,
                                         float eps, float wd, float w1, float b2, float w2, float gscale) {
    g *= gscale;
    if (wd != 0.f) g = g + wd * p;
    m = m + w1 * (g - m);
    v = v * b2 + (w2 * g) * g;
    const float denom = sqrtf(v) / bc2_sqrt + eps;
    p = p + (-step_size) * (m / denom);
}

__device__ __forceinline__ int any_halt(const int32_t* halt, int n_halt) {
    int bad = 0;
    for (int i = 0; i < n_halt; ++i)
        bad |= __hip_atomic_load(halt + 2 * i, __ATOMIC_RELAXED, __HIP_MEMORY_SCOPE_AGENT) != 0;
    return bad;
}

struct AdamGate {
    int32_t* flag;
    const int32_t* ctr;
    int add;
    int32_t* err;
    int max_spins;
    int64_t lo, hi;
};

__global__ __launch_bounds__(256) void adam_kernel(float* __restrict__ p, const float* __restrict__ g,
                                                   float* __restrict__ m, float* __restrict__ v, int64_t n, float lr,
                                                   float b1, float b2, float eps, float wd, float gscale,
                                                   const int32_t* __restrict__ step_dev, int vec4, AdamGate gate,
                                                   const int32_t* __restrict__ halt, int n_halt) {
    __shared__ float sc[2];
    __shared__ int halted;
    bool need = false;
    if (gate.flag != nullptr) {
        const int64_t per = vec4 ? 4 : 1, span = (int64_t)blockDim.x * per;
        const int64_t bstride = (int64_t)gridDim.x * span;
        need = gate.hi > (vec4 ? ((n >> 2) << 2) : n) && gate.lo < n;
        for (int64_t e0 = blockIdx.x * span; e0 < n; e0 += bstride) need = need || (e0 < gate.hi && e0 + span > gate.lo);
    }
    if (threadIdx.x == 0) {
        int want = 0, seen = 0;
        if (need) {
            want = gate.ctr[0] + gate.add;
            seen = __hip_atomic_load(gate.flag, __ATOMIC_ACQUIRE, __HIP_MEMORY_SCOPE_AGENT);
        }
        int h = any_halt(halt, n_halt);
        adam_consts(lr, b1, b2, step_dev, &sc[0], &sc[1]);
        if (need && seen - want < 0) {
            const long long t0 = wall_clock64();
            int k = 0;
            while (__hip_atomic_load(gate.flag, __ATOMIC_ACQUIRE, __HIP_MEMORY_SCOPE_AGENT) - want < 0) {
                __builtin_amdgcn_s_sleep(4);
                if (++k > gate.max_spins) {
                    atomicExch(gate.err, 1);
                    break;
                }
            }
            atomicAdd(gate.err + 1, (int32_t)(wall_clock64() - t0));
            h = h || any_halt(halt, n_halt);
        }
        halted = h;
    }
    if (need) {
        __syncthreads();
        __builtin_amdgcn_fence(__ATOMIC_ACQUIRE, "agent");
    }
    __syncthreads();
    if (halted) return;
    const float step_size = sc[0], bc2_sqrt = sc[1];
    const float w1 = (float)(1.0 - (double)b1), w2 = (float)(1.0 - (double)b2);
    const int64_t stride = (int64_t)gridDim.x * blockDim.x;
    const int64_t t0 = blockIdx.x * (int64_t)blockDim.x + threadIdx.x;
    if (vec4) {
        const int64_t n4 = n >> 2;
        float4* p4 = reinterpret_cast<float4*>(p);
        const float4* g4 = reinterpret_cast<const float4*>(g);
        float4* m4 = reinterpret_cast<float4*>(m);
        float4* v4 = reinterpret_cast<float4*>(v);
        for (int64_t i = t0; i < n4; i += stride) {
            float4 pp = p4[i], gg = g4[i], mm = m4[i], vv = v4[i];
            adam_one(pp.x, gg.x, mm.x, vv.x, step_size, bc2_sqrt, eps, wd, w1, b2, w2, gscale);
            adam_one(pp.y, gg.y, mm.y, vv.y, step_size, bc2_sqrt, eps, wd, w1, b2, w2, gscale);
            adam_one(pp.z, gg.z, mm.z, vv.z, step_size, bc2_sqrt, eps, wd, w1, b2, w2, gscale);
            adam_one(pp.w, gg.w, mm.w, vv.w, step_size, bc2_sqrt, eps, wd, w1, b2, w2, gscale);
            p4[i] = pp;
            m4[i] = mm;
            v4[i] = vv;
        }
        for (int64_t i = (n4 << 2) + t0; i < n; i += stride)
            adam_one(p[i], g[i], m[i], v[i], step_size, bc2_sqrt, eps, wd, w1, b2, w2, gscale);
    } else {
        for (int64_t i = t0; i < n; i += stride)
            adam_one(p[i], g[i], m[i], v[i], step_size, bc2_sqrt, eps, wd, w1, b2, w2, gscale);
    }
}

typedef float adam_f4 __attribute__((ext_vector_type(4)));
__global__ __launch_bounds__(256) void adam_stream_kernel(float* __restrict__ p, const float* __restrict__ g,
                                                          float* __restrict__ m, float* __restrict__ v, int64_t n, float lr,
                                                          float b1, float b2, float eps, float wd, float gscale,
                                                          const int32_t* __restrict__ step_dev,
                                                          const int32_t* __restrict__ halt, int n_halt) {
    __shared__ float sc[2];
    __shared__ int halted;
    if (threadIdx.x == 0) {
        adam_consts(lr, b1, b2, step_dev, &sc[0], &sc[1]);
        halted = any_halt(halt, n_halt);
    }
    __syncthreads();
    if (halted) return;
    const float step_size = sc[0], bc2_sqrt = sc[1];
    const float w1 = (float)(1.0 - (double)b1), w2 = (float)(1.0 - (double)b2);
    const int64_t stride = (int64_t)gridDim.x * blockDim.x, n4 = n >> 2;
    const int64_t t0 = blockIdx.x * (int64_t)blockDim.x + threadIdx.x;
    adam_f4* p4 = reinterpret_cast<adam_f4*>(p);
    const adam_f4* g4 = reinterpret_cast<const adam_f4*>(g);
    adam_f4* m4 = reinterpret_cast<adam_f4*>(m);
    adam_f4* v4 = reinterpret_cast<adam_f4*>(v);
    for (int64_t i = t0; i < n4; i += 2 * stride) {
        adam_f4 pp[2], gg[2], mm[2], vv[2];
#pragma unroll
        for (int u = 0; u < 2; ++u) {
            const int64_t j = i + u * stride < n4 ? i + u * stride : i;
            pp[u] = __builtin_nontemporal_load(p4 + j);
            gg[u] = __builtin_nontemporal_load(g4 + j);
            mm[u] = __builtin_nontemporal_load(m4 + j);
            vv[u] = __builtin_nontemporal_load(v4 + j);
        }
#pragma unroll
        for (int u = 0; u < 2; ++u) {
#pragma unroll
            for (int e = 0; e < 4; ++e) {
                float a = pp[u][e], b = mm[u][e], c = vv[u][e];
                adam_one(a, gg[u][e], b, c, step_size, bc2_sqrt, eps, wd, w1, b2, w2, gscale);
                pp[u][e] = a; mm[u][e] = b; vv[u][e] = c;
            }
            const int64_t j = i + u * stride;
            if (j < n4) {
                __builtin_nontemporal_store(pp[u], p4 + j);
                __builtin_nontemporal_store(mm[u], m4 + j);
                __builtin_nontemporal_store(vv[u], v4 + j);
            }
        }
    }
    for (int64_t i = (n4 << 2) + t0; i < n; i += stride)
        adam_one(p[i], g[i], m[i], v[i], step_size, bc2_sqrt, eps, wd, w1, b2, w2, gscale);
}

__global__ void counter_add_kernel(int32_t* c, int n_words, int64_t inc) {
    if (threadIdx.x != 0 || blockIdx.x != 0) return;
    if (n_words == 1) {
        c[0] = (int32_t)(c[0] + inc);
    } else {
        uint64_t v = ((uint64_t)(uint32_t)c[1] << 32) | (uint32_t)c[0];
        v += (uint64_t)inc;
        c[0] = (int32_t)(uint32_t)v;
        c[1] = (int32_t)(uint32_t)(v >> 32);
    }
}

__global__ void counters_add2_kernel(int32_t* c1, int n1, int64_t inc1, int32_t* c2, int n2, int64_t inc2, dv_publish pub) {
    if (threadIdx.x != 0 || blockIdx.x != 0) return;
    publish_block0(pub);
    int32_t* cs[2] = {c1, c2};
    const int ns[2] = {n1, n2};
    const int64_t incs[2] = {inc1, inc2};
    for (int t = 0; t < 2; ++t) {
        int32_t* c = cs[t];
        if (ns[t] == 1) {
            c[0] = (int32_t)(c[0] + incs[t]);
        } else {
            uint64_t v = ((uint64_t)(uint32_t)c[1] << 32) | (uint32_t)c[0];
            v += (uint64_t)incs[t];
            c[0] = (int32_t)(uint32_t)v;
            c[1] = (int32_t)(uint32_t)(v >> 32);
        }
    }
// ... 269 lines not shown
```

drvae_amd/engine.py:

```python
import math
import os
from collections import OrderedDict
from dataclasses import dataclass, field
from typing import List, Optional, Tuple

import numpy as np
import torch

from . import kernels as K
from . import tuning as T
from ._lib import GAUSS_LOGVAR, GAUSS_SIGMA
from .arena import N_LOSS, ParamArena, span
from .chain import _Chain, _Lin, _pad4
from .plan import LOSS_IDX, _Plan
from .schedule import DUAL, EVAL, FORK_JOIN, StepSchedule, StepSync, _Branch



@dataclass
class StepConfig:
    kind: str = 'drvae'
    dim_x: int = 978
    dim_y: int = 2
    dim_z1: int = 100
# ... 548 lines not shown
            QYm = p.c_clf.forward(clf_in)
            K.rows_gather(p.FPIN[:, :Z1], Z1blk, p.fp_src)
            K.ycont_fwd(p.YLrow, p.FPIN[:, Z1:], p.Z3IN[:, Z3:], QYm, p.ylab, p.has_y_i32, p.EY, Y_LOGVAR_CONT, B,
                        sqerr=cfg.kind == 'vfae')
            Q3 = p.c_top.forward([p.FPIN])
            K.kl_rows_fwd(p.KL3, p.KL3raw, Q3[:, :Z3], Q3[:, Z3:], prior=(0.0, 0.0), free_bits=True,
                          kl_min=cfg.kl_min, eps=p.E3, zout=p.Z3IN[:, :Z3])
            PZ1 = p.c_dz1.forward([p.Z3IN])
            K.kl_rows_fwd(p.KLDrow, p.KL1raw, Qmu, Qlv, PZ1[:, :Z1], PZ1[:, Z1:], qidx=p.fp_q, free_bits=True,
                          kl_min=cfg.kl_min, add=p.KL3)
            return
        if cfg.has_y:
            if p.Mf:
                Z3, Y = cfg.dim_z3, cfg.dim_y
                if not self._fprop_from_heads():
                    K.rows_gather(p.FPIN, Z1blk, p.fp_src, onehot_cls=p.fp_cls, n_classes=Y)
                if self.fuse_heads and (self.fuse_bwd or p.Mf < 8192):
                    Q3 = p.c_top.forward([p.FPIN], heads=dict(sample=dict(eps=p.E3, out=p.Z3IN[:, :Z3], n_src=p.Mf)))
                    PZ1 = p.c_dz1.forward([p.Z3IN])
                    if not self._fprop_tail():
                        K.kl_rows_fwd(p.KLFP, p.KL1raw, Qmu, Qlv, PZ1[:, :Z1], PZ1[:, Z1:], qidx=p.fp_q,
                                      free_bits=True, kl_min=cfg.kl_min, prior=(0.0, 0.0),
                                      second=(Q3[:, :Z3], Q3[:, Z3:], p.KL3raw))
                else:
                    Q3 = p.c_top.forward([p.FPIN])
                    K.kl_rows_fwd(p.KL3, p.KL3raw, Q3[:, :Z3], Q3[:, Z3:], prior=(0.0, 0.0), free_bits=True,
                                  kl_min=cfg.kl_min, eps=p.E3, zout=p.Z3IN[:, :Z3])
                    PZ1 = p.c_dz1.forward([p.Z3IN])
                    K.kl_rows_fwd(p.KLFP, p.KL1raw, Qmu, Qlv, PZ1[:, :Z1], PZ1[:, Z1:], qidx=p.fp_q, free_bits=True,
                                  kl_min=cfg.kl_min, add=p.KL3)
        klz2_here = cfg.has_pert and Np and not self._tail.klz2_on_main
        clf_park = (mid_park is not None and not klz2_here and cfg.has_y and self.clf_small
                    and (L * B + 3) // 4 <= 256)
        fold_mid = mid_park is not None and klz2_here and (L * Np + 3) // 4 <= 256
        if mid is not None and not fold_mid and not clf_park:
            mid()
        if klz2_here:
            P2 = p.c_z2F.out[-1]
            K.kl_rows_fwd(p.KLZ2, p.KLZ2raw, Qmu, Qlv, P2[:, :Z1], P2[:, Z1:], qidx=p.qz2_idx, pidx=p.pidx,
                          reps=L, free_bits=True, kl_min=cfg.kl_min, park=mid_park if fold_mid else None)
        if cfg.has_y:
            if cfg.kind == 'drvae':
                clf_in = [Z1blk, p.D] if cfg.clf_z1z2 else [p.Z2F]
            else:
                clf_in = [Z1blk]
            ym = (p.YLrow, p.KLDrow, p.CFP, p.DQY, p.label_r, p.fp_ptr, p.KLFP, p.log_prior, p.c_kld, p.c_yl)
            if self.clf_small:
                lc = self.L_clf[0]
                fk = None
                if self._fprop_tail():
                    fk = dict(Q=p.c_enc.out[-1], qidx=p.fp_q, P=p.c_dz1.out[-1], Q3=p.c_top.out[-1], Z1=Z1,
                              Z3=cfg.dim_z3, kl_min=cfg.kl_min, raw1=p.KL1raw, raw3=p.KL3raw, dq=p.DQFP, dp=p.DPZ1)
                K.smalln_fwd(p.QY, None, clf_in[0], lc.W, lc.b, clf_in[1] if len(clf_in) > 1 else None,
                             ymarg=ym if self.fuse_bwd else None, park=mid_park if clf_park else None, fprop_kl=fk)
            else:
                K.softmax_clamp_fwd(p.QY, p.c_clf.forward(clf_in), sigmoid1=cfg.clf_1sig)
            if self.fuse_bwd and self.clf_small:
                pass
            elif self.fuse_bwd:
                K.ymarg_fwdbwd(p.YLrow, p.KLDrow, p.CFP, p.DQY, p.QY, p.label_r, p.fp_ptr, p.KLFP, p.log_prior,
                               p.c_kld, p.c_yl)
            else:
                K.ymarg_fwd(p.YLrow, p.KLDrow, p.QY, p.label_r, p.fp_ptr, p.KLFP, p.log_prior)

    def join_side(self):
        if self._side_graph is not None and self.dev.type == 'cuda':
            torch.cuda.current_stream().wait_stream(self.flag_side)

    def _dual_capable(self, on_gpu=None):
        cfg = self.cfg
        if cfg.has_y:
            return self.branch.on if on_gpu is None else bool(self.concurrent and on_gpu)
        return bool(cfg.kind == 'pvae' and self.concurrent and cfg.optim_alg == 'adam')

    def _side_adam_layout(self):
        heads = self.L_decx[-1]
        g0 = self.arena.grad.storage_offset()
        hs = min(heads.dW.storage_offset(), heads.db.storage_offset()) - g0
        ok = bool(len(self.L_decx) > 1 and heads.g is None and hs % 4 == 0 and self.arena.n_live == self.arena.n_params
                  and max(heads.dW.storage_offset() + span(heads.dW),
                          heads.db.storage_offset() + heads.db.numel()) - g0 >= self.arena.n_live - 3)
        return ok, hs

    def sync_side_counters(self):
        self.side_ctr.copy_(self.step_dev)
        self.side_t.copy_(self.step_dev + 1)
        self.sync.flag('tail').copy_(self.step_dev)

    def _fprop_from_heads(self):
        cfg, p = self.cfg, self.plan
        return bool(self.fuse_heads and self._heads_small(p.DPX) and cfg.has_y and not cfg.cont and p.Mf)

    def _fprop_tail(self):
        cfg, p = self.cfg, self.plan
        return bool(self.fuse_bwd and self.fuse_heads and self.clf_small and cfg.has_y and not cfg.cont and p.Mf)

    def _mmd_penalty(self):
        cfg, p = self.cfg, self.plan
        if p.mmd_grouped is not None:
            g = p.mmd_grouped
            if g['W'] is not None:
                g['W'].normal_()
                g['b'].uniform_()
            K.mmd_grouped_fwd(g)
            K.mmd_grouped_bwd(g)
            return
        if cfg.kernel_MMD in ('rbf_fourier', 'identity') and getattr(p, 'mmd_items', None) and T.get('mmd_explicit'):
            return self._mmd_penalty_launches()
        from . import blocks as blk
        with torch.enable_grad():
            z = p.ZDEC[:p.o3].detach().clone().requires_grad_(True)
            total = z.new_zeros(())
            for rows, sind, pairs in p.mmd_calls:
                total = total + blk.mmd_criterion(z.index_select(0, rows), sind, cfg.kernel_MMD, pairs=pairs) / cfg.L
            total.backward()
        p.MMDval.copy_(total.detach().reshape(1))
        p.DZMMD.copy_(z.grad * (-cfg.mmd_rate / p.n_tot))

    def _mmd_penalty_launches(self):
        cfg, p = self.cfg, self.plan
        Z, rff = cfg.dim_z1, cfg.kernel_MMD == 'rbf_fourier'
        R = 500
        a, c = math.sqrt(2. / 2.) / math.sqrt(Z), math.sqrt(2. / R)
        z = p.ZDEC[:p.o3]
        dev = z.device
        bufs = p.__dict__.get('_mmd_bufs')
        if bufs is None:
            f = lambda *shape: torch.zeros(*shape, device=dev)
            nmax = max(it['n0'] + it['n1'] for it in p.mmd_items)
            bufs = p._mmd_bufs = dict(zz=f(nmax, _pad4(Z))[:, :Z], dz=f(nmax, _pad4(Z))[:, :Z], diff=f(R if rff else Z), m2=f(1),
                                      rs=f(1), g=f(1))
            if rff:
                bufs.update(th=f(nmax, R), G=f(nmax, R), W=f(Z, R), b=f(R), bias=f(R), scale=torch.full((R,), a, device=dev))
        B_ = bufs
        p.DZMMD.zero_()
        p.MMDval.zero_()
        fac = -cfg.mmd_rate / p.n_tot
        for it in p.mmd_items:
            n0, n1 = it['n0'], it['n1']
            n = n0 + n1
            zz, dz = B_['zz'][:n], B_['dz'][:n]
            K.rows_gather(zz, z, it['idx32'])
            if rff:
                th, G = B_['th'][:n], B_['G'][:n]
                B_['W'].normal_()
                B_['b'].uniform_()
                torch.mul(B_['b'], 2 * math.pi, out=B_['bias'])
                K.gemm(th, zz, B_['W'], True, False, epi=K.EPI_FWD, scale=B_['scale'], bias=B_['bias'])
                K.mmd_rff_fwd(B_['diff'], B_['m2'], th[:n0], th[n0:], c)
            else:
                K.mmd_identity_fwd(B_['diff'], B_['m2'], zz[:n0], zz[n0:])
            torch.rsqrt(B_['m2'], out=B_['rs'])
            p.MMDval.addcmul_(B_['m2'], B_['rs'], value=-it['w'])
            torch.mul(B_['rs'], -0.5 * it['w'] * fac, out=B_['g'])
            if rff:
                K.mmd_rff_bwd(G[:n0], th[:n0], B_['diff'], B_['g'], 2.0 * c / n0)
                K.mmd_rff_bwd(G[n0:], th[n0:], B_['diff'], B_['g'], -2.0 * c / n1)
                K.gemm(dz, G, B_['W'], True, True, alpha=a)
            else:
                K.mmd_identity_bwd(dz[:n0], B_['diff'], B_['g'], 2.0 / n0)
                K.mmd_identity_bwd(dz[n0:], B_['diff'], B_['g'], -2.0 / n1)
            p.DZMMD.index_add_(0, it['idx'], dz)

    def _loss_scalars(self, after=None, terms_elsewhere=False, bump_counters=False):
        cfg, p = self.cfg, self.plan
        L = cfg.L
        nll = p.NLLP if self._nll_fused else (p.NLLC if self._nll_cs else p.NLL)
        rl = nll.shape[1] if nll.dim() == 2 else 1
        if p.universal:
            terms = [(nll[:p.o3], p.w_recl[:p.o3], 1.0, 0, rl)]
            if cfg.has_pert:
                terms.append((nll[p.o3:], p.w_pert[:L * p.Np], 1.0, 2, rl))
                terms.append((p.KLZ2, p.c_klz2, 1.0, 1))
        else:
            terms = [(nll[:p.o3], None, 1.0 / (L * p.n_tot), 0)]
            if cfg.has_pert and p.Np:
                terms.append((nll[p.o3:], None, 1.0 / (L * max(1., p.n_pairs)), 2))
                terms.append((p.KLZ2, p.c_klz2, 1.0, 1))
        if cfg.kind == 'pvae':
            terms.append((p.KLP, p.c_klp, 1.0, 1) if p.universal else (p.KLP, None, 1.0 / p.n_tot, 1))
        if cfg.has_y:
            terms.append((p.KLDrow, None, 1.0 / (L * p.n_tot), 1))
            terms.append((p.YLrow, p.w_yl, 1.0, 3) if p.universal else
                         (p.YLrow, None, 1.0 / (L * max(1., p.n_lab)), 3))
        if p.DZMMD is not None:
            terms.append((p.MMDval, None, 1.0 / p.n_tot, 4))
        bump = ()
        if after is not None or bump_counters:
            bump = [(self.step_dev, 1)] + ([(self.rng_ctr, self._rng_pending)] if self._rng_pending else [])
            self._rng_pending = 0
            self._ctr_bumped = True
        K.loss_assemble(self.arena.loss, [] if terms_elsewhere else terms, p.w_elbo, p.w_cmpl, after=after, bump=bump,
                        halt=self.sync_err, accum=self.loss_sum if self.fuse_bwd else None)

    def backward(self):
        cfg, p = self.cfg, self.plan
        B, Np, L, Z1, X = p.B, p.Np, cfg.L, cfg.dim_z1, cfg.dim_x
        Q = p.c_enc.out[-1]
        Qmu, Qlv = Q[:, :Z1], Q[:, Z1:]
        DQ = p.DQ
        Z1blk, DZ1 = p.ZDEC[:L * B], p.DZDEC[:L * B]
        mode, t = self._mode(), self._tail
        late, leaf = t.late, []

        PX = p.c_decx.out[-1]
        if not self.fuse_bwd and cfg.type_rec != 'diag_gaussian':
            K.rec_nll_rows(p.NLL, p.XIN, PX, kind=cfg.type_rec, shift=REC_ACT[cfg.type_rec][1], xidx=p.tgt, coef=p.c_nll,
                           dpre=p.DPX)
        elif not self.fuse_bwd:
            K.nll_rows_bwd(p.DPX[:, :X], p.DPX[:, X:], p.c_nll, p.XIN, PX[:, :X], PX[:, X:], mode=GAUSS_SIGMA,
                           xidx=p.tgt, sd_act='softplus', sd_shift=1e-3)
        if mode == DUAL and self._rec == 'side':
            self._side_backward(Qmu, Qlv, Z1blk, late, leaf)
            self._side_graph_tail(leaf)
            return
        if mode == EVAL:
            self.branch.fork()
        elif mode == FORK_JOIN:
            self.branch._forked = True
        p.c_decx.backward(p.DPX, p.dec_in, [[(p.DZDEC, 1.0, 0.0)]] + [None] * (len(p.dec_in) - 1),
                          publish_after_last=self.sync.pub('rows', self.step_dev) if t.side_loss else None,
                          db_last_done=bool(self.fuse_bwd and self._nll_cs))
        if p.DZMMD is not None:
            p.DZDEC[:p.o3].add_(p.DZMMD)
        if self._after_decoder_bwd is not None:
            self._after_decoder_bwd()
        if mode != DUAL:
            with self.branch:
                self._side_backward(Qmu, Qlv, Z1blk, late, leaf)
            self.branch.join()
        park = bump = None
        if t.fold_join:
            park = self.sync.wait('join', self.step_dev)
            bump = [(self.step_dev, 1)] + ([(self.rng_ctr, self._rng_pending)] if self._rng_pending else [])
            self._rng_pending = 0
            self._ctr_bumped = True
        elif mode == DUAL:
            self._loss_scalars(after=self.sync.wait('join', self.step_dev), terms_elsewhere=t.side_loss)
        elif mode == FORK_JOIN:
            self._loss_scalars(bump_counters=True)
        if t.adam_gated:
            if cfg.has_y:
                lc, g0 = self.L_clf[0], self.arena.grad.storage_offset()
                lo = min(lc.dW.storage_offset(), lc.db.storage_offset()) - g0
                hi = max(lc.dW.storage_offset() + span(lc.dW), lc.db.storage_offset() + lc.db.numel()) - g0
            else:
                lo, hi = 0, 4
            self._adam_gate = self.sync.gate('clf_dw' if t.tail_gated else 'tail', self.step_dev, lo, hi)
            self._adam_n = t.hs if t.side_adam else None
        if t.cap_fork:
            self._adam_gate = self.sync.gate('tail', self.step_dev, 0, 4)
        if cfg.has_pert:
            P2 = p.c_z2F.out[-1]
            K.z2f_post_bwd(p.DP2, DZ1, DQ[B:] if Np else None, p.DZ2F if cfg.has_y else None,
                           p.DZDEC[p.o3:] if Np else None, p.pair_slot,
                           p.E2F, P2, Q[B:] if Np else None, p.c_klz2, p.KLZ2raw, cfg.kl_min,
                           p.DZ1B if cfg.has_y else None, L, B, Np, park=park,
                           prior=(p.c_klp[B:], p.KLPraw[B:]) if (cfg.kind == 'pvae' and Np) else None)
            p.c_z2F.backward(p.DP2, [Z1blk], [[(DZ1, 1.0, 1.0)]])
        add1 = p.DZ1B if (cfg.has_y and not cfg.has_pert) else None
        fp = cfg.has_y and p.Mf
        K.reparam_bwd_seg(DQ[:B, :Z1], DQ[:B, Z1:], p.DZDEC, p.E12, Qlv, p.zseg_ptr, p.zseg_rows,
                          extra=p.DQFP if fp else None, ex_ptr=p.q_ptr if fp else None,
                          ex_rows=p.q_rows if fp else None, bump=bump, dz_add=add1,
                          prior=(p.c_klp, p.KLPraw, cfg.kl_min, Qmu) if cfg.kind == 'pvae' else None)
        p.c_enc.backward(DQ, p.enc_in, None,
                         publish_first=self.sync.pub('noise', self.step_dev, 0) if t.noise_ahead else None)

    def _side_backward(self, Qmu, Qlv, Z1blk, late, leaf):
        cfg, p = self.cfg, self.plan
        B, Np, L, Z1 = p.B, p.Np, cfg.L, cfg.dim_z1

        def wgrad_clf(*args):
            ws = getattr(p, 'SNWS', None)
            if late:
                leaf.append(lambda pub=None: K.smalln_bwd_weight(*args, publish=pub, ws=ws))
            else:
                K.smalln_bwd_weight(*args, ws=ws)

        if cfg.has_y and cfg.cont:
            Y, Z3 = cfg.dim_y, cfg.dim_z3
            PZ1, Q3, QYm = p.c_dz1.out[-1], p.c_top.out[-1], p.c_clf.out[-1]
            K.ycont_bwd(None, p.CFP, QYm, p.ylab, p.has_y_i32, Y_LOGVAR_CONT, p.c_yl, p.c_kld, p.DFPIN[:, Z1:],
                        p.DZ3IN[:, Z3:], B, sqerr=cfg.kind == 'vfae')
            K.kl_rows_bwd(p.DQFP[:, :Z1], p.DQFP[:, Z1:], p.DPZ1[:, :Z1], p.DPZ1[:, Z1:], p.CFP, p.KL1raw,
                          Qmu, Qlv, PZ1[:, :Z1], PZ1[:, Z1:], qidx=p.fp_q, free_bits=True, kl_min=cfg.kl_min)
            p.c_dz1.backward(p.DPZ1, [p.Z3IN], [[(p.DZ3IN, 1.0, 0.0)]])
            K.kl_rows_bwd(p.DQ3[:, :Z3], p.DQ3[:, Z3:], None, None, p.CFP, p.KL3raw, Q3[:, :Z3], Q3[:, Z3:],
                          prior=(0.0, 0.0), free_bits=True, kl_min=cfg.kl_min, dz=p.DZ3IN[:, :Z3], eps=p.E3)
            p.c_top.backward(p.DQ3, [p.FPIN], [[(p.DFPIN, 1.0, 0.0)]])
            K.rows_segment_sum(p.DZ1B, p.DFPIN, seg_ptr=p.fp_ptr, beta=0.0, width=Z1)
            K.ycont_bwd(p.DLOG, None, QYm, p.ylab, p.has_y_i32, Y_LOGVAR_CONT, p.c_yl, p.c_kld, p.DFPIN[:, Z1:],
                        p.DZ3IN[:, Z3:], B, sqerr=cfg.kind == 'vfae')
            if cfg.kind == 'drvae' and cfg.clf_z1z2:
                p.c_clf.backward(p.DLOG, [Z1blk, p.D], [[(p.DZ1B, 1.0, 1.0)], [(p.DZ2F, 1.0, 0.0), (p.DZ1B, -1.0, 1.0)]])
            elif cfg.kind == 'drvae':
                p.c_clf.backward(p.DLOG, [p.Z2F], [[(p.DZ2F, 1.0, 0.0)]])
            else:
                p.c_clf.backward(p.DLOG, [Z1blk], [[(p.DZ1B, 1.0, 1.0)]])
        elif cfg.has_y:
            Y = cfg.dim_y
            if not self.fuse_bwd:
                K.ymarg_bwd(p.CFP, p.DQY, p.QY, p.label_r, p.fp_ptr, p.KLFP, p.log_prior, p.c_kld, p.c_yl)
            if p.Mf:
                Z3 = cfg.dim_z3
                PZ1, Q3 = p.c_dz1.out[-1], p.c_top.out[-1]
                if not self._fprop_tail():
                    K.kl_rows_bwd(p.DQFP[:, :Z1], p.DQFP[:, Z1:], p.DPZ1[:, :Z1], p.DPZ1[:, Z1:], p.CFP, p.KL1raw,
                                  Qmu, Qlv, PZ1[:, :Z1], PZ1[:, Z1:], qidx=p.fp_q, free_bits=True,
                                  kl_min=cfg.kl_min)
                klq = dict(out=p.DQ3, q=Q3, eps=p.E3, coef=p.CFP, raw=p.KL3raw, kl_min=cfg.kl_min, Z=Z3) \
                    if self.fuse_bwd else None
                if not p.c_dz1.backward(p.DPZ1, [p.Z3IN], [[(p.DZ3IN, 1.0, 0.0)]], klq=klq):
                    K.kl_rows_bwd(p.DQ3[:, :Z3], p.DQ3[:, Z3:], None, None, p.CFP, p.KL3raw, Q3[:, :Z3], Q3[:, Z3:],
                                  prior=(0.0, 0.0), free_bits=True, kl_min=cfg.kl_min, dz=p.DZ3IN[:, :Z3], eps=p.E3)
                p.c_top.backward(p.DQ3, [p.FPIN], [[(p.DFPIN, 1.0, 0.0)]])
                seg_in_clf = self.clf_small and not (cfg.kind == 'drvae' and not cfg.clf_z1z2)
                if not seg_in_clf:
                    K.rows_segment_sum(p.DZ1B, p.DFPIN, seg_ptr=p.fp_ptr, beta=0.0, width=Z1)
            b1 = 1.0 if p.Mf else 0.0
            seg = (p.DFPIN, p.fp_ptr) if p.Mf else None
            two = cfg.kind == 'drvae' and cfg.clf_z1z2
            if self.clf_small:
                lc = self.L_clf[0]
                if two:
                    K.smalln_bwd_data([(p.DZ1B, 0, 1.0, b1, Z1, -1.0), (p.DZ2F, Z1, 1.0, 0.0)], p.DQY, p.QY, lc.W,
                                      seg=seg)
                    wgrad_clf(lc.dW, lc.db, p.DQY, p.QY, Z1blk, p.D)
                elif cfg.kind == 'drvae':
                    K.smalln_bwd_data([(p.DZ2F, 0, 1.0, 0.0)], p.DQY, p.QY, lc.W)
                    wgrad_clf(lc.dW, lc.db, p.DQY, p.QY, p.Z2F)
                    if not p.Mf:
                        p.DZ1B.zero_()
                else:
                    K.smalln_bwd_data([(p.DZ1B, 0, 1.0, b1)], p.DQY, p.QY, lc.W, seg=seg)
                    wgrad_clf(lc.dW, lc.db, p.DQY, p.QY, Z1blk)
            else:
                K.softmax_clamp_bwd(p.DLOG, p.DQY, p.QY, sigmoid1=cfg.clf_1sig)
                if two:
                    p.c_clf.backward(p.DLOG, [Z1blk, p.D],
                                     [[(p.DZ1B, 1.0, b1)], [(p.DZ2F, 1.0, 0.0), (p.DZ1B, -1.0, 1.0)]])
                elif cfg.kind == 'drvae':
                    p.c_clf.backward(p.DLOG, [p.Z2F], [[(p.DZ2F, 1.0, 0.0)]])
                    if not p.Mf:
                        p.DZ1B.zero_()
                else:
                    p.c_clf.backward(p.DLOG, [Z1blk], [[(p.DZ1B, 1.0, b1)]])

    def _side_graph_tail(self, leaf):
        cfg, p, t, sync, ctr = self.cfg, self.plan, self._tail, self.sync, self.side_ctr
        if leaf:
            leaf[0](pub=sync.pub('join', ctr))
            for fn in leaf[1:]:
                fn()
        else:
            K.flag_publish(*sync.pub('join', ctr))
        if t.side_loss:
            a, hs = self.arena, t.hs
            K.flag_wait(*sync.wait('rows', ctr), publish=sync.pub('clf_dw', ctr) if t.tail_gated else None)
            if t.side_adam:
                K.adam_l2(a.param[hs:a.n_live], a.grad[hs:a.n_live], a.exp_avg[hs:a.n_live],
                          a.exp_avg_sq[hs:a.n_live], self.side_t, lr=cfg.learning_rate,
                          weight_decay=cfg.weight_decay, halt=self.sync_err)
            self._loss_scalars()
        if t.noise_ahead:
            K.flag_wait(*sync.wait('noise', ctr))
            K.fill_normal_rows(p.noise, p.noise_desc, self.seed, self.rng_ctr)
        K.counters_add2(ctr, 1, self.side_t, 1, publish=sync.pub('tail', ctr) if (t.late or t.cap_fork) else None)

    def optimizer_step(self, gscale=1.0):
        cfg, a = self.cfg, self.arena
        if self._ctr_bumped:
            self._ctr_bumped = False
        elif self._rng_pending:
            K.counters_add2(self.step_dev, 1, self.rng_ctr, self._rng_pending)
            self._rng_pending = 0
        else:
            K.counter_add(self.step_dev, 1)
        if self._rec == 'both' and self.sched == 5 and self._dual_capable():
            K.counters_add2(self.side_ctr, 1, self.side_t, 1, publish=self.sync.pub('tail', self.side_ctr))
        step = K.adamax_l2 if cfg.optim_alg == 'adamax' else K.adam_l2
        n = a.n_live
        if self._adam_n is not None:
            n, self._adam_n = self._adam_n, None
        kw = {}
        if self._adam_gate is not None:
            kw['gate'], self._adam_gate = self._adam_gate, None
        step(a.param[:n], a.grad[:n], a.exp_avg[:n], a.exp_avg_sq[:n], self.step_dev, lr=cfg.learning_rate,
             weight_decay=cfg.weight_decay, gscale=gscale, halt=self.sync_err, **kw)

    def train_step(self, noise=None, allreduce=None):
        self.training = True
        self.join_side()
        if noise is not None:
            self.set_noise(noise)
        else:
            self.draw_noise(bump=False)
        self._launch_sequence(allreduce=allreduce, draw=False)
        self.iters += 1

    def losses(self):
        self.join_side()
        v = self.arena.loss.detach().cpu().tolist()
        if self._side_graph is not None:
            self.check_sync()
        keys = ['RECL', 'KLD', 'PERT', 'YL', 'MMD', 'ELBO', 'CMPL']
        if self.cfg.kind == 'pvae':
            keys.remove('YL')
        if self.cfg.kind == 'vfae':
            keys.remove('PERT')
        return OrderedDict((k, v[LOSS_IDX[k]]) for k in keys)
```

drvae_amd/kernels.py:

```python
import ctypes as C
import os
from typing import Any, NamedTuple, Optional

import torch

from . import _lib
from ._lib import ACT, EPI_BWD, EPI_FWD, EPI_KLQ, EPI_PLAIN, GAUSS_LOGVAR, GAUSS_SIGMA, GemmDesc


def _stream():
    return C.c_void_p(torch.cuda.current_stream().cuda_stream)


def _f32(t, name='tensor'):
    if t is None:
        return None
    if not (t.is_cuda and t.dtype == torch.float32):
        raise RuntimeError('drvae_amd kernels need CUDA/HIP float32 tensors (%s is %s on %s); there is no CPU '
                           'fallback' % (name, t.dtype, t.device))
    if t.dim() >= 1 and t.numel() > 0 and t.stride(-1) != 1 and t.size(-1) != 1:
        raise RuntimeError('%s must have unit inner stride' % name)
    return t.data_ptr()


# ... 718 lines not shown
        assert part.dtype == torch.float64 and part.is_cuda and part.is_contiguous() and tuple(part.shape[1:]) == (3, X)
    else:
        assert out.dtype == torch.float64 and out.is_cuda and out.is_contiguous() and tuple(out.shape) == (3, X)
        nb = col_moment_blocks(M)
        part = out.unsqueeze(0) if nb == 1 else torch.empty(nb, 3, X, dtype=torch.float64, device=out.device)
    _lib.check(_lib.load().dv_col_moments(_f32(x), _ld(x), _f32(r), _ld(r), M, X, part.data_ptr(), nb, _i32(sel), _f32(r_bias), _stream()),
               'dv_col_moments')
    if out is not None and part.data_ptr() != out.data_ptr():
        torch.sum(part, 0, out=out)


def col_moment_blocks(M):
    return max(1, min(64, max(min(16, (M + 255) // 256), (M + 511) // 512)))


RECON_ROWS_MAX_X = 1024


def recon_rows(rows, ll, x, mu, sd, *, bias=None, sd_shift=1e-3):
    M, X = x.shape
    assert tuple(mu.shape) == (M, X) and tuple(sd.shape) == (M, X) and _ld(mu) == _ld(sd)
    assert rows.is_contiguous() and tuple(rows.shape) == (M, 6)
    d = _lib.ReconRows(x=_f32(x), ldx=_ld(x), mu=_f32(mu), sd=_f32(sd), ldp=_ld(mu),
                       bias_mu=_f32(bias[0]) if bias is not None else None,
                       bias_sd=_f32(bias[1]) if bias is not None else None, sd_shift=sd_shift, M=M, X=X,
                       rows=_f32(rows), ll=_f32(ll))
    _lib.check(_lib.load().dv_recon_rows(C.byref(d), _stream()), 'dv_recon_rows')


def recon_finalize(out4, rows, part, X, *, sel=None, n=None, ll=None):
    n = (sel.numel() if sel is not None else rows.shape[0]) if n is None else n
    assert out4.dtype == torch.float64 and out4.is_cuda and out4.numel() >= 4 and out4.is_contiguous()
    assert part.dtype == torch.float64 and part.is_contiguous() and rows.is_contiguous() and rows.shape[1] == 6
    _lib.check(_lib.load().dv_recon_finalize(_f32(rows), _i32(sel), n, X, part.data_ptr(), part.shape[0], _f32(ll),
                                             out4.data_ptr(), _stream()), 'dv_recon_finalize')


RANK_MAX_ROWS = 32768


def rank_metrics(out, counts, proba, y32, *, pred32=None, sel=None, c0=1, n_cls=1, binary=True):
    n = sel.numel() if sel is not None else proba.shape[0]
    assert out.dtype == torch.float64 and out.is_cuda and out.numel() >= 2 * n_cls + 1 and out.is_contiguous()
    assert counts.dtype == torch.int32 and counts.is_contiguous() and counts.numel() >= n_cls * n * 4
    _lib.check(_lib.load().dv_rank_metrics(_f32(proba), _ld(proba), _i32(y32), _i32(pred32), _i32(sel), n, c0, n_cls,
                                           int(bool(binary)), counts.data_ptr(), out.data_ptr(), _stream()), 'dv_rank_metrics')


def loss_assemble(loss, terms, w_elbo, w_cmpl, after=None, bump=(), halt=None, accum=None):
    hp, hn = _halt(halt)
    arr = (_lib.LossTerm * max(len(terms), 1))()
    for i, term in enumerate(terms):
        x, w, scale, out = term[:4]
        arr[i].x, arr[i].w, arr[i].n, arr[i].scale, arr[i].out = _f32(x), _f32(w), x.numel(), scale, out
        arr[i].row_len = term[4] if len(term) > 4 else 1
    if after is None and not bump:
        _lib.check(_lib.load().dv_loss_assemble(arr, len(terms), _f32(w_elbo), _f32(w_cmpl), _f32(loss), hp, hn,
                                                _f32(accum), _stream()), 'dv_loss_assemble')
    else:
        _lib.check(_lib.load().dv_loss_assemble_after(_wait(after), arr, len(terms), _f32(w_elbo), _f32(w_cmpl), _f32(loss),
                                                      _bump(bump), hp, hn, _f32(accum), _stream()), 'dv_loss_assemble_after')


def axpby(y, x, a=1.0, b=0.0):
    assert x.is_contiguous() and y.is_contiguous() and x.numel() == y.numel()
    _lib.check(_lib.load().dv_axpby(_f32(x), a, _f32(y), b, x.numel(), _stream()), 'dv_axpby')


def adam_l2(p, g, m, v, step_dev, *, lr, beta1=0.9, beta2=0.999, eps=1e-8, weight_decay=0.0, gscale=1.0, gate=None,
            halt=None):
    assert p.is_contiguous() and g.is_contiguous() and m.is_contiguous() and v.is_contiguous()
    hp, hn = _halt(halt)
    h = _lib.AdamHyper(lr=lr, beta1=beta1, beta2=beta2, eps=eps, weight_decay=weight_decay, gscale=gscale)
    if gate is None:
        _lib.check(_lib.load().dv_adam_l2(_f32(p), _f32(g), _f32(m), _f32(v), p.numel(), C.byref(h), _i32(step_dev), hp, hn,
                                          _stream()), 'dv_adam_l2')
    else:
        gate = Gate(*gate)
        _lib.check(_lib.load().dv_adam_l2_gated(_f32(p), _f32(g), _f32(m), _f32(v), p.numel(), C.byref(h), _i32(step_dev),
                                                _wait(Wait(gate.flag, gate.ctr, gate.err, gate.add)), gate.lo, gate.hi, hp, hn,
                                                _stream()), 'dv_adam_l2_gated')


def adamax_l2(p, g, m, u, step_dev, *, lr, beta1=0.9, beta2=0.999, eps=1e-8, weight_decay=0.0, gscale=1.0, halt=None):
    assert p.is_contiguous() and g.is_contiguous() and m.is_contiguous() and u.is_contiguous()
    hp, hn = _halt(halt)
    h = _lib.AdamHyper(lr=lr, beta1=beta1, beta2=beta2, eps=eps, weight_decay=weight_decay, gscale=gscale)
    _lib.check(_lib.load().dv_adamax_l2(_f32(p), _f32(g), _f32(m), _f32(u), p.numel(), C.byref(h), _i32(step_dev), hp, hn,
                                        _stream()), 'dv_adamax_l2')


def flag_publish(flag, ctr, add=1):
    _lib.check(_lib.load().dv_flag_publish(_i32(flag), _i32(ctr), add, _stream()), 'dv_flag_publish')


WAIT_SPINS = int(os.environ.get('DRVAE_WAIT_SPINS', '4000000'))


def flag_wait(flag, ctr, err, add=1, max_spins=None, publish=None):
    max_spins = WAIT_SPINS if max_spins is None else max_spins
    _lib.check(_lib.load().dv_flag_wait(_i32(flag), _i32(ctr), add, _i32(err), max_spins, _publish(publish), _stream()),
               'dv_flag_wait')


def counter_add(counter, inc=1):
    _lib.check(_lib.load().dv_counter_add(_i32(counter), counter.numel(), inc, _stream()), 'dv_counter_add')


def counters_add2(c1, inc1, c2, inc2, publish=None):
    _lib.check(_lib.load().dv_counters_add2(_i32(c1), c1.numel(), inc1, _i32(c2), c2.numel(), inc2, _publish(publish),
                                            _stream()), 'dv_counters_add2')


def fill_normal_rows(arena, desc, seed, ctr_dev=None, park=None):
    assert arena.is_contiguous() and desc.dim() == 2 and desc.shape[1] == 4
    _lib.check(_lib.load().dv_fill_normal_rows(_f32(arena), _i32(desc), desc.shape[0], seed, _i32(ctr_dev), _wait(park),
                                               _stream()), 'dv_fill_normal_rows')


def fill_normal(out, seed, ctr_dev=None):
    assert out.is_contiguous()
    _lib.check(_lib.load().dv_fill_normal(_f32(out), out.numel(), seed, _i32(ctr_dev), _stream()),
               'dv_fill_normal')
```

drvae_amd/schedule.py:

```python
import contextlib
import ctypes
import gc
import os
import weakref
from typing import NamedTuple

import torch

from . import kernels as K
from . import tuning as T


def _masked_stream(bits, device):
    hip = ctypes.CDLL('libamdhip64.so')
    st = ctypes.c_void_p()
    arr = (ctypes.c_uint32 * len(bits))(*bits)
    with torch.cuda.device(device):
        rc = hip.hipExtStreamCreateWithCUMask(ctypes.byref(st), len(bits), arr)
    if rc != 0:
        raise RuntimeError('hipExtStreamCreateWithCUMask failed: %d' % rc)
    import atexit

    def _destroy(handle=st.value):
        try:
            torch.cuda.synchronize()
            hip.hipStreamDestroy(ctypes.c_void_p(handle))
        except Exception:
            pass
    atexit.register(_destroy)
    return torch.cuda.ExternalStream(st.value, device=device)


SYNC_POLL = 64

EVAL, FORK_JOIN, DUAL = 'evaluation pass', 'one graph with a fork/join', 'one chain of the dual-graph step'

FLAGS = (
    ('z1', 'main', True),
    ('join', 'side', False),
    ('z2f', 'main', True),
    ('tail', 'side', True),
    ('rows', 'main', False),
    ('noise', 'main', False),
    ('clf_dw', 'side', False),
    ('unused', None, False),
)
SITES = (
    ('join', 'main', ('join',)),
    ('z1', 'side', ('z1',)),
    ('z2f', 'side', ('z2f',)),
    ('adam_gate', 'main', ('tail', 'clf_dw')),
    ('rows', 'side', ('rows',)),
    ('noise', 'side', ('noise',)),
    ('next_step', 'main', ('tail',)),
)
FLAG_INDEX = {f[0]: i for i, f in enumerate(FLAGS)}
SITE_INDEX = {s[0]: i for i, s in enumerate(SITES)}


class StepSync:

    def __init__(self, device):
        self.flags = torch.zeros(len(FLAGS), dtype=torch.int32, device=device)
        self.err = torch.zeros(2 * len(SITES), dtype=torch.int32, device=device)

    def flag(self, name):
        return self.flags[FLAG_INDEX[name]:FLAG_INDEX[name] + 1]

    def pub(self, name, ctr, add=1):
        return K.Publish(self.flag(name), ctr, add)

    def wait(self, site, ctr, add=1, max_spins=None, flag=None):
        i, flags = SITE_INDEX[site], SITES[SITE_INDEX[site]][2]
        assert flag is None or flag in flags, (site, flag)
        return K.Wait(self.flag(flag or flags[0]), ctr, self.err[2 * i:2 * i + 2], add, max_spins)

    def gate(self, flag, ctr, lo, hi):
        w = self.wait('adam_gate', ctr, 0, flag=flag)
        return K.Gate(w.flag, w.ctr, w.add, w.err, lo, hi)


class Tail(NamedTuple):
    dual: bool = False
    late: bool = False
    adam_gated: bool = False
    side_adam: bool = False
    hs: int = 0
    side_loss: bool = False
    cap_fork: bool = False
    tail_gated: bool = False
    noise_ahead: bool = False
    klz2_on_main: bool = False
    fold_join: bool = False

_PINNED_POOL = []
_PARTITION_STREAMS = {}


class _Branch:

    def __init__(self, device, enabled=True):
        self.on = enabled and torch.device(device).type == 'cuda'
        self.side = torch.cuda.Stream(device=device) if self.on else None
        self._forked = False

    def fork(self):
        if self.on:
            self.side.wait_stream(torch.cuda.current_stream())
            self._forked = True

    def __enter__(self):
        if self.on:
            if not self._forked:
                self.side.wait_stream(torch.cuda.current_stream())
            self._forked = False
            self._ctx = torch.cuda.stream(self.side)
            self._ctx.__enter__()
        return self

    def __exit__(self, *exc):
        if self.on:
            self._ctx.__exit__(*exc)

    def join(self):
        if self.on:
            torch.cuda.current_stream().wait_stream(self.side)


_CAPTURE_STATE = ('_graphs', '_side_graph', 'noise_ahead', '_graph_key', '_graph_feed', '_graph_mmd_sig',
                  '_captured_allreduce', '_graph_noise')


class StepSchedule:

    def _init_schedule_state(self):
        self._graphs = []
        self._side_graph = None
        self.noise_ahead = False
        self._graph_key = None
        self._graph_feed = None
        self._graph_mmd_sig = None
        self._captured_allreduce = None
        self._graph_noise = None
        self._captures = {}
        self._rec = 'both'
        self._tail = Tail()
        self._late_fork = False
        self._after_decoder_bwd = None
        self._nll_fused = False
        self._nll_cs = False
        self._rng_pending = 0
        self._ctr_bumped = False
        self._adam_n = None
        self._adam_gate = None
        self._noise_stale = True
        self._flag_side = None
        self._flags_ok = None
        self._side_cus = None
        self._since_poll = 0
        self._sync_host = None
        self._sync_event = None

    def stash_capture(self):
        assert self._graph_key == self.plan.key, 'stash_capture right after capture(): another plan is current'
        self._captures[self.plan.key] = {k: getattr(self, k) for k in _CAPTURE_STATE}

    def use_capture(self, key):
        cap = self._captures.get(key)
        if cap is None or cap['_graph_feed'] is not self._plans[key].live_feed or \
                cap['_graph_noise'] not in (None, self.add_noise):
            return False
        if self._graph_key != key:
            for k, v in cap.items():
                setattr(self, k, v)
            self.plan = self._plans[key]
            self._noise_stale = True
        return True

    def _mode(self):
        return EVAL if not self.fuse_bwd else DUAL if self._rec != 'both' else FORK_JOIN

    def _step_tail(self, split_kind, on_gpu=None):
        cfg, p = self.cfg, self.plan
        if not (self.sched == 5 and self._dual_capable(on_gpu) and self._latency_bound() and
                (self._flags_usable() if on_gpu is None else on_gpu) and (cfg.has_y or not split_kind)):
            return Tail()
        late_ok = bool(not cfg.cont and cfg.optim_alg == 'adam' and (self.clf_small if cfg.has_y else True))
        late = late_ok and split_kind in (False, True)
        side_ok, hs = self._side_adam_layout()
        side_adam = late and not split_kind and side_ok
        cap_fork = bool(split_kind == 'captured' and side_ok and late_ok and cfg.has_y and T.get('dp_fork'))
        side_loss = side_adam or (late and split_kind is True and len(self.L_decx) > 1)
        tail_gated = side_adam and (p.live_feed is not None or T.get('tail_gate') == 2)
        klz2_on_main = not cfg.cont and cfg.has_y and not (p.universal and len(p.key) <= 3)
        fold_join = side_loss and cfg.has_pert and (p.B * cfg.dim_z1 + 255) // 256 <= 256
        return Tail(dual=True, late=late, adam_gated=late and not split_kind, side_adam=side_adam, hs=hs, side_loss=side_loss,
                    cap_fork=cap_fork, tail_gated=tail_gated, noise_ahead=late or cap_fork, klz2_on_main=klz2_on_main,
                    fold_join=fold_join)

    @contextlib.contextmanager
    def _recording(self, chain, tail):
        self._rec, self._tail = chain, tail
        try:
            yield
        finally:
            self._rec, self._tail = 'both', Tail()

    def _launch_sequence(self, allreduce=None, draw=True, optimizer=True):
        self.fuse_bwd = True
        try:
            if draw:
                self.draw_noise(bump=False)
            self.forward()
            self.backward()
            if optimizer and allreduce is not None:
                allreduce(self.arena.xchg)
        finally:
            self.fuse_bwd = False
        if optimizer:
            self.optimizer_step()

    def capture(self, split_for_allreduce=False, allreduce=None):
        self._captured_allreduce = allreduce if split_for_allreduce == 'captured' else None
        assert self.plan is not None, 'set_batch first'
        self.join_side()
        if self.plan.DZMMD is not None and split_for_allreduce:
            raise NotImplementedError('use_MMD: the model-level MMD penalty is a cross-row term (every row of a nuisance '
                                      'class against every other row): it cannot be sharded over ranks')
        self.training = True
        self.plan.set_beta(self.beta_pert())
        side = torch.cuda.Stream()
        side.wait_stream(torch.cuda.current_stream())
        with torch.cuda.stream(side):
            self.draw_noise(bump=False)
            self._rng_pending = 0
            self.forward()
            self.backward()
        torch.cuda.current_stream().wait_stream(side)
        torch.cuda.synchronize()
        self._graphs = []
        self._side_graph = None
        tail = self._step_tail(split_for_allreduce)
        self.noise_ahead = tail.noise_ahead
        self._noise_stale = True
        gc.collect()
        gc_was_on = gc.isenabled()
        gc.disable()
        self._late_fork = self.branch.on and not tail.dual and not self._latency_bound()
        try:
            with self._recording('main', tail) if tail.dual else contextlib.nullcontext():
                self._capture_main(split_for_allreduce)
            if tail.dual:
                self.sync_side_counters()
                self.flag_side.wait_stream(torch.cuda.current_stream())
                gs = torch.cuda.CUDAGraph()
                with torch.cuda.graph(gs, stream=self.flag_side), self._recording('side', tail):
                    self._launch_sequence(draw=False, optimizer=False)
                self._side_graph = gs
        finally:
            self._late_fork = False
            if gc_was_on:
                gc.enable()
        self._graph_key = self.plan.key
        self._graph_feed = self.plan.live_feed
        self._graph_mmd_sig = getattr(self.plan, 'mmd_sig', None)
        return self

    def _latency_bound(self):
        return self.plan is not None and self.plan.DPX.shape[0] * self.plan.DPX.shape[1] <= (4 << 20)

    def _partition_applicable(self):
        small = self._latency_bound()
        if not self.cfg.has_y and self._side_graph is None:
            return False
        return bool(self.sched == 5 and self._dual_capable() and small and
                    int(os.environ.get('DRVAE_SIDE_CUS', '64')) > 0)

    def _part_streams(self, n_side):
        cache = _PARTITION_STREAMS.setdefault(torch.device(self.dev).index or 0, {})
        n_side = int(n_side)
        if n_side not in cache:
# ... 210 lines not shown
```

drvae_amd/tuning.py:

```python
import os

DEFAULTS = {
    'sched': 5,
    'fuse_heads': 1,
    'raw_heads': 1,
    'tail_gate': 1,
    'concurrent': 1,
    'nll_cs': 1,
    'mmd_explicit': 1,
    'dp_fork': 1,
}

CHOICES = {'sched': (3, 5), 'fuse_heads': (0, 1), 'raw_heads': (1, 2), 'tail_gate': (1, 2), 'concurrent': (0, 1),
           'nll_cs': (1, 2), 'mmd_explicit': (0, 1), 'dp_fork': (0, 1)}


def _parse():
    out = dict(DEFAULTS)
    for kv in filter(None, os.environ.get('DRVAE_TUNE', '').split(',')):
        k, _, v = kv.partition('=')
        k = k.strip()
        if k not in DEFAULTS:
            raise ValueError('DRVAE_TUNE: unknown switch %r (known: %s)' % (k, ', '.join(sorted(DEFAULTS))))
        out[k] = int(v)
        if out[k] not in CHOICES[k]:
            raise ValueError('DRVAE_TUNE: %s=%d is not a schedule (known: %s)' % (k, out[k], CHOICES[k]))
    return out


_VALUES = None


def get(name):
    global _VALUES
    if _VALUES is None:
        _VALUES = _parse()
    return _VALUES[name]


def reload():
    global _VALUES
    _VALUES = None
```

include/drvae_hip.h:

```cpp
#ifndef DRVAE_HIP_H
#define DRVAE_HIP_H

#include <stdint.h>

#ifdef __cplusplus
extern "C" {
#endif

typedef void* dv_stream_t;

#define DV_ABI_VERSION 12

enum { DV_OK = 0, DV_ERR_ARG = -1, DV_ERR_LAUNCH = -2, DV_ERR_UNSUPPORTED = -3 };

enum {
    DV_ACT_IDENTITY = 0, DV_ACT_ELU = 1, DV_ACT_SOFTPLUS = 2, DV_ACT_SIGMOID = 3, DV_ACT_TANH = 4,
    DV_ACT_RELU = 5, DV_ACT_LEAKY_RELU = 6, DV_ACT_SELU = 7, DV_ACT_SOFTSIGN = 8, DV_ACT_COS = 9
};

enum { DV_GAUSS_LOGVAR = 0, DV_GAUSS_SIGMA = 1 };

enum { DV_EPI_PLAIN = 0, DV_EPI_FWD = 1, DV_EPI_BWD = 2, DV_EPI_KLQ = 3 };

int dv_abi_version(void);
// ... 431 lines not shown
int dv_mmd_identity_bwd(const float* diff, const float* gout, float coef, int32_t n, int32_t Z, float* dx, int64_t ldd,
                        dv_stream_t stream);

int dv_nuisance_feed(const int32_t* s, const int32_t* table, int32_t n_batches, const int32_t* ctr, const int32_t* base,
                     int32_t B, const int32_t* pair_rows, int32_t Np, int32_t L, int32_t S, float* sohe, int64_t lde,
                     float* sohd, int64_t ldd, int32_t* cls, dv_stream_t stream);
#define DV_MMD_MAX_CLASSES 8
typedef struct dv_mmd_grouped_desc {
    const float* z;
    int64_t ldz;
    int32_t n_z;
    int32_t Z;
    int32_t kind;
    int32_t R;
    int32_t n_groups;
    int32_t n_entries;
    int32_t max_rows;
    int32_t S;
    int32_t B;
    const int32_t* grp_ptr;
    const int32_t* rows;
    const int32_t* src;
    const int32_t* cls;
    const float* W;
    const float* b;
    float a;
    float c;
    float w;
    float fac;
    float* theta;
    float* diff;
    int32_t* cnt;
    float* m2;
    float* value;
    float* dz;
    int64_t ldd;
} dv_mmd_grouped_desc;
int dv_mmd_grouped_fwd(const dv_mmd_grouped_desc* d, dv_stream_t stream);
int dv_mmd_grouped_bwd(const dv_mmd_grouped_desc* d, dv_stream_t stream);

#define DV_RANK_MAX_ROWS 32768
int dv_recon_finalize(const float* rows, const int32_t* sel, int32_t n, int32_t X, const double* cols, int32_t row_blocks,
                      const float* ll, double* out, dv_stream_t stream);
int dv_rank_metrics(const float* proba, int64_t ldp, const int32_t* y, const int32_t* pred, const int32_t* sel, int32_t n,
                    int32_t c0, int32_t n_cls, int32_t binary, int32_t* counts, double* out, dv_stream_t stream);

#define DV_MAX_LOSS_TERMS 8
typedef struct dv_loss_term {
    const float* x;
    const float* w;
    int32_t n;
    float scale;
    int32_t out;
    int32_t row_len;
} dv_loss_term;
int dv_loss_assemble(const dv_loss_term* terms, int32_t n_terms, const float* w_elbo, const float* w_cmpl,
                     float* loss, const int32_t* halt, int32_t n_halt, float* accum, dv_stream_t stream);
int dv_loss_assemble_after(const dv_wait* wait, const dv_loss_term* terms, int32_t n_terms, const float* w_elbo,
                           const float* w_cmpl, float* loss, const dv_bump* bump, const int32_t* halt, int32_t n_halt,
                           float* accum, dv_stream_t stream);
int dv_bn_fwd(const float* x, int64_t ldx, int32_t M, int32_t N, const float* w, const float* b, float eps,
              float* mean_out, float* rstd_out, float* y, int64_t ldy, float* running_mean, float* running_var,
              float momentum, int32_t training, dv_stream_t stream);
int dv_bn_bwd(const float* dy, int64_t ldd, const float* x, int64_t ldx, const float* mean, const float* rstd,
              const float* w, int32_t M, int32_t N, float* dx, int64_t lddx, float* dw, float* db, int32_t training,
              dv_stream_t stream);
int dv_mask_scale(const float* x, int64_t ldx, const float* mask, int64_t ldm, float scale, int32_t M, int32_t N,
                  float* y, int64_t ldy, dv_stream_t stream);
int dv_axpby(const float* x, float a, float* y, float b, int64_t n, dv_stream_t stream);

typedef struct dv_adam_hyper {
    float lr;
    float beta1;
    float beta2;
    float eps;
    float weight_decay;
    float gscale;
} dv_adam_hyper;
int dv_adam_l2(float* p, const float* g, float* m, float* v, int64_t n, const dv_adam_hyper* h,
               const int32_t* step_dev, const int32_t* halt, int32_t n_halt, dv_stream_t stream);
int dv_adam_l2_gated(float* p, const float* g, float* m, float* v, int64_t n, const dv_adam_hyper* h,
                     const int32_t* step_dev, const dv_wait* gate, int64_t lo, int64_t hi, const int32_t* halt,
                     int32_t n_halt, dv_stream_t stream);
int dv_adamax_l2(float* p, const float* g, float* m, float* u, int64_t n, const dv_adam_hyper* h,
                 const int32_t* step_dev, const int32_t* halt, int32_t n_halt, dv_stream_t stream);
int dv_counter_add(int32_t* counter_lo_hi, int32_t n_words, int64_t inc, dv_stream_t stream);
int dv_counters_add2(int32_t* c1, int32_t n1, int64_t inc1, int32_t* c2, int32_t n2, int64_t inc2,
                     const dv_publish* pub, dv_stream_t stream);

int dv_flag_publish(int32_t* flag, const int32_t* ctr, int32_t add, dv_stream_t stream);
int dv_flag_wait(int32_t* flag, const int32_t* ctr, int32_t add, int32_t* err, int32_t max_spins, const dv_publish* pub,
                 dv_stream_t stream);

int dv_fill_normal(float* out, int64_t n, uint64_t seed, const int32_t* ctr_dev, dv_stream_t stream);
int dv_fill_normal_rows(float* arena, const int32_t* desc, int32_t n_rows, uint64_t seed, const int32_t* ctr_dev,
                        const dv_wait* park, dv_stream_t stream);

#ifdef __cplusplus
}
#endif
#endif
```

Before: 1.641 million samples/s.

## Fuse Adam update into first encoder weight-gradient GEMM epilogue with sweep workgroups

Adds a combined kernel that computes the first encoder layer's weight/bias gradient GEMM and applies the Adam update directly in its epilogue. Spare workgroups in the same launch sweep the rest of the main-stream optimizer slice, gated on the side chain's flag. The separate main-path Adam launch is skipped, and the parameter/moment loads are overlapped with the GEMM pipeline fill. This removes a kernel launch and the gradient round trip through memory for the largest layer. In exchange it adds register pressure in the GEMM, extra spin-gating in sweep blocks, and a repartition of the optimizer range between streams.

```diff
diff --git a/drvae_amd/_lib.py b/drvae_amd/_lib.py
--- a/drvae_amd/_lib.py
+++ b/drvae_amd/_lib.py
@@ -204,6 +204,8 @@
     'dv_axpby': [_p, _f, _p, _f, _i64, _p],
     'dv_adam_l2': [_p, _p, _p, _p, _i64, C.POINTER(AdamHyper), _p, _p, _i32, _p],
     'dv_adam_l2_gated': [_p, _p, _p, _p, _i64, C.POINTER(AdamHyper), _p, C.POINTER(Wait), _i64, _i64, _p, _i32, _p],
+    'dv_gemm_dw_adam': [C.POINTER(GemmDesc), _p, _p, _p, _p, _i64, C.POINTER(AdamHyper), _p, _i64, _i64, C.POINTER(Wait), _i64, _i64,
+                        _p, _i32, _i32, _p],
     'dv_adamax_l2': [_p, _p, _p, _p, _i64, C.POINTER(AdamHyper), _p, _p, _i32, _p],
     'dv_flag_publish': [_p, _p, _i32, _p],
     'dv_flag_wait': [_p, _p, _i32, _p, _i32, C.POINTER(Publish), _p],
diff --git a/drvae_amd/chain.py b/drvae_amd/chain.py
--- a/drvae_amd/chain.py
+++ b/drvae_amd/chain.py
@@ -89,7 +89,7 @@
         return self.out[-1]
 
     def backward(self, dpre_last, inputs, dinputs=None, publish_after_last=None, publish_first=None, db_last_done=False,
-                 klq=None):
+                 klq=None, first_dw=None):
         dpre = dpre_last
         pending_pub = publish_first
         took_klq = False
@@ -128,8 +128,12 @@
             c0 = 0
             for si, s in enumerate(srcs):
                 w = s.shape[1]
-                K.linear_bwd_weight(dW[:, c0:c0 + w], dpre, s, dbias=db if si == 0 else None, overread=True,
-                                    npad=len(srcs) == 1 and l.g is None and self._pad_ok(s))
+                wgrad = K.linear_bwd_weight
+                if li == 0 and first_dw is not None:
+                    assert len(srcs) == 1 and l.g is None and dinputs is None
+                    wgrad = first_dw
+                wgrad(dW[:, c0:c0 + w], dpre, s, dbias=db if si == 0 else None, overread=True,
+                      npad=len(srcs) == 1 and l.g is None and self._pad_ok(s))
                 c0 += w
             if l.g is not None:
                 K.wn_bwd(l.dW, l.dg, l.raw, l.W, l.g, l.norm)
diff --git a/drvae_amd/csrc/adam_common.inc b/drvae_amd/csrc/adam_common.inc
--- /dev/null
+++ b/drvae_amd/csrc/adam_common.inc
@@ -0,0 +1,105 @@
+
+__device__ __forceinline__ void adam_consts(float lr, float b1, float b2, const int32_t* step_dev, float* step_size,
+                                            float* bc2_sqrt) {
+    const double t = (double)step_dev[0];
+    const double bc1 = 1.0 - pow((double)b1, t);
+    const double bc2 = 1.0 - pow((double)b2, t);
+    *step_size = (float)((double)lr / bc1);
+    *bc2_sqrt = (float)sqrt(bc2);
+}
+
+__device__ __forceinline__ void adam_one(float& p, float g, float& m, float& v, float step_size, float bc2_sqrt,
+                                         float eps, float wd, float w1, float b2, float w2, float gscale) {
+#pragma clang fp contract(off)
+    g *= gscale;
+    if (wd != 0.f) g = __builtin_fmaf(wd, p, g);
+    m = __builtin_fmaf(w1, g - m, m);
+    v = __builtin_fmaf(w2 * g, g, v * b2);
+    const float denom = sqrtf(v) / bc2_sqrt + eps;
+    p = __builtin_fmaf(-step_size, m / denom, p);
+}
+
+__device__ __forceinline__ int any_halt(const int32_t* halt, int n_halt) {
+    int bad = 0;
+    for (int i = 0; i < n_halt; ++i)
+        bad |= __hip_atomic_load(halt + 2 * i, __ATOMIC_RELAXED, __HIP_MEMORY_SCOPE_AGENT) != 0;
+    return bad;
+}
+
+struct AdamGate {
+    int32_t* flag;
+    const int32_t* ctr;
+    int add;
+    int32_t* err;
+    int max_spins;
+    int64_t lo, hi;
+};
+
+__device__ __forceinline__ void adam_sweep_block(float* __restrict__ p, const float* __restrict__ g, float* __restrict__ m,
+                                                 float* __restrict__ v, int64_t n, float lr, float b1, float b2, float eps,
+                                                 float wd, float gscale, const int32_t* __restrict__ step_dev, int vec4,
+                                                 const AdamGate& gate, const int32_t* __restrict__ halt, int n_halt,
+                                                 int64_t bid, int64_t nblk, float* sc, int* halted) {
+    bool need = false;
+    if (gate.flag != nullptr) {
+        const int64_t per = vec4 ? 4 : 1, span = (int64_t)blockDim.x * per;
+        const int64_t bstride = nblk * span;
+        need = gate.hi > (vec4 ? ((n >> 2) << 2) : n) && gate.lo < n;
+        for (int64_t e0 = bid * span; e0 < n; e0 += bstride) need = need || (e0 < gate.hi && e0 + span > gate.lo);
+    }
+    if (threadIdx.x == 0) {
+        int want = 0, seen = 0;
+        if (need) {
+            want = gate.ctr[0] + gate.add;
+            seen = __hip_atomic_load(gate.flag, __ATOMIC_ACQUIRE, __HIP_MEMORY_SCOPE_AGENT);
+        }
+        int h = any_halt(halt, n_halt);
+        adam_consts(lr, b1, b2, step_dev, &sc[0], &sc[1]);
+        if (need && seen - want < 0) {
+            const long long t0 = wall_clock64();
+            int k = 0;
+            while (__hip_atomic_load(gate.flag, __ATOMIC_ACQUIRE, __HIP_MEMORY_SCOPE_AGENT) - want < 0) {
+                __builtin_amdgcn_s_sleep(4);
+                if (++k > gate.max_spins) {
+                    atomicExch(gate.err, 1);
+                    break;
+                }
+            }
+            atomicAdd(gate.err + 1, (int32_t)(wall_clock64() - t0));
+            h = h || any_halt(halt, n_halt);
+        }
+        *halted = h;
+    }
+    if (need) {
+        __syncthreads();
+        __builtin_amdgcn_fence(__ATOMIC_ACQUIRE, "agent");
+    }
+    __syncthreads();
+    if (*halted) return;
+    const float step_size = sc[0], bc2_sqrt = sc[1];
+    const float w1 = (float)(1.0 - (double)b1), w2 = (float)(1.0 - (double)b2);
+    const int64_t stride = nblk * blockDim.x;
+    const int64_t t0 = bid * (int64_t)blockDim.x + threadIdx.x;
+    if (vec4) {
+        const int64_t n4 = n >> 2;
+        float4* p4 = reinterpret_cast<float4*>(p);
+        const float4* g4 = reinterpret_cast<const float4*>(g);
+        float4* m4 = reinterpret_cast<float4*>(m);
+        float4* v4 = reinterpret_cast<float4*>(v);
+        for (int64_t i = t0; i < n4; i += stride) {
+            float4 pp = p4[i], gg = g4[i], mm = m4[i], vv = v4[i];
+            adam_one(pp.x, gg.x, mm.x, vv.x, step_size, bc2_sqrt, eps, wd, w1, b2, w2, gscale);
+            adam_one(pp.y, gg.y, mm.y, vv.y, step_size, bc2_sqrt, eps, wd, w1, b2, w2, gscale);
+            adam_one(pp.z, gg.z, mm.z, vv.z, step_size, bc2_sqrt, eps, wd, w1, b2, w2, gscale);
+            adam_one(pp.w, gg.w, mm.w, vv.w, step_size, bc2_sqrt, eps, wd, w1, b2, w2, gscale);
+            p4[i] = pp;
+            m4[i] = mm;
+            v4[i] = vv;
+        }
+        for (int64_t i = (n4 << 2) + t0; i < n; i += stride)
+            adam_one(p[i], g[i], m[i], v[i], step_size, bc2_sqrt, eps, wd, w1, b2, w2, gscale);
+    } else {
+        for (int64_t i = t0; i < n; i += stride)
+            adam_one(p[i], g[i], m[i], v[i], step_size, bc2_sqrt, eps, wd, w1, b2, w2, gscale);
+    }
+}
diff --git a/drvae_amd/csrc/gemm.hip b/drvae_amd/csrc/gemm.hip
--- a/drvae_amd/csrc/gemm.hip
+++ b/drvae_amd/csrc/gemm.hip
@@ -3,6 +3,23 @@
 namespace {
 
 #include "gemm_pipe.inc"
+#include "adam_common.inc"
+
+struct DwAdam {
+    float* p;
+    const float* g;
+    float* m;
+    float* v;
+    float lr, b1, b2, eps, wd, gscale;
+    const int32_t* step_dev;
+    const int32_t* halt;
+    int n_halt;
+};
+struct DwSweep {
+    int64_t lo2, n2;
+    int vec4;
+    AdamGate gate;
+};
 
 
 struct Operand {
@@ -143,9 +160,12 @@
     return 2 * stage > red ? 2 * stage : red;
 }
 
-template <int BM, int BN, int BK, int WM, int WN, int KS, bool AKC, bool BKC, bool PAIR = false, bool MI16 = false, int PS = 0>
+template <int BM, int BN, int BK, int WM, int WN, int KS, bool AKC, bool BKC, bool PAIR = false, bool MI16 = false, int PS = 0,
+          bool ADAM = false>
 __device__ __forceinline__ void gemm_body(const dv_gemm_desc& g, const LoadCfg& lc, float* smem, int bid, int nwg,
-                                          const dv_heads_epi* he = nullptr) {
+                                          const dv_heads_epi* he = nullptr, const DwAdam* da = nullptr, float* ad_sc = nullptr,
+                                          int* ad_halted = nullptr) {
+    static_assert(!ADAM || (PS > 0 && KS > 1 && !PAIR && !MI16), "optimiser epilogue: the K-split pipe tilings");
     static_assert(!PAIR || (AKC && BKC && KS > 1 && WM == 1 && WN == 1), "paired heads: forward layout, K-split tiling");
     constexpr int HB = BN / 2;
     static_assert(!MI16 || (KS == 1 && !PAIR), "16x16x4 tiles: unsplit K only");
@@ -338,7 +358,37 @@
     const int nkt = (g.K + BK - 1) / BK, nfull = g.K / BK;
     float* const buf0 = smem;
     float* const buf1 = smem + STAGE;
-    if constexpr (PS > 0) {
+    constexpr int ARPT = ADAM ? BM / (NT / BN) : 1;
+    [[maybe_unused]] float ad_p[ARPT], ad_m[ARPT], ad_v[ARPT];
+    [[maybe_unused]] auto ad_index = [&](int e) -> int64_t {
+        const int row = m0 + (tid / BN) * ARPT + e, col = n0 + tid % BN;
+        if (row >= g.M) return -1;
+        if (ones_col && col == g.N + DV_ONES_OFF(g)) return (g.a_colsum - da->g) + row;
+        if (col < g.N) return (g.C - da->g) + (int64_t)row * g.ldc + col;
+        return -1;
+    };
+    if constexpr (PS > 0 && ADAM) {
+        int ad_h = 0, ad_t = 0;
+        if (tid == 0) {
+            ad_h = any_halt(da->halt, da->n_halt);
+            ad_t = da->step_dev[0];
+        }
+#pragma unroll
+        for (int e = 0; e < ARPT; ++e) {
+            const int64_t i = ad_index(e), ic = i < 0 ? (int64_t)(g.C - da->g) : i;
+            ad_p[e] = da->p[ic];
+            ad_m[e] = da->m[ic];
+            ad_v[e] = da->v[ic];
+        }
+        pipe_loop<BM, BN, BK, WM, WN, KS, PS, AKC, BKC, (BM < 128 && !AKC && !BKC)>(
+            g, smem, m0, n0, [&](int l) { return m0 + l < g.M ? m0 + l : g.M - 1; }, bline, acc, [&]() {
+                if (tid == 0) {
+                    adam_consts(da->lr, da->b1, da->b2, &ad_t, &ad_sc[0], &ad_sc[1]);
+                    *ad_halted = ad_h;
+                }
+            });
+        __syncthreads();
+    } else if constexpr (PS > 0) {
         if (!(DV_DBG & 64))
             pipe_loop<BM, BN, BK, WM, WN, KS, PS, AKC, BKC, (BM < 128 && !AKC && !BKC)>(
                 g, smem, m0, n0, [&](int l) { return m0 + l < g.M ? m0 + l : g.M - 1; }, bline, acc);
@@ -554,6 +604,23 @@
         }
         const int rbase = m0 + r0;
         epi_store_col<RPT>(g, a4, n0 + col, [rbase](int r) { return rbase + r; });
+        if constexpr (ADAM) {
+            if (*ad_halted) return;
+            const float step_size = ad_sc[0], bc2_sqrt = ad_sc[1];
+            const float w1 = (float)(1.0 - (double)da->b1), w2 = (float)(1.0 - (double)da->b2);
+            const bool on_ones = ones_col && n0 + col == g.N + DV_ONES_OFF(g);
+#pragma unroll
+            for (int e = 0; e < RPT; ++e) {
+                const int64_t i = ad_index(e);
+                const float gv = on_ones ? 0.f + a4[e] : a4[e] * g.alpha;
+                adam_one(ad_p[e], gv, ad_m[e], ad_v[e], step_size, bc2_sqrt, da->eps, da->wd, w1, da->b2, w2, da->gscale);
+                if (i >= 0) {
+                    da->p[i] = ad_p[e];
+                    da->m[i] = ad_m[e];
+                    da->v[i] = ad_v[e];
+                }
+            }
+        }
     }
 }
 
@@ -790,6 +857,22 @@
     gemm_body<BM, BN, BK, BM / 32, BN / 32, KS, AKC, BKC, false, false, PS>(g, lc, smem, blockIdx.x, gridDim.x);
 }
 
+template <int BK, int WPS>
+__global__ __launch_bounds__(256, WPS) void gemm_dw_adam_kernel(const dv_gemm_desc g, const LoadCfg lc, const DwAdam da, const DwSweep sw,
+                                                                int tiles) {
+    __shared__ __attribute__((aligned(1024))) float smem[gemm_smem_floats<32, 32, BK, 4, false, false, 2>()];
+    __shared__ float sc[2];
+    __shared__ int halted;
+    publish_on_entry(g);
+    if ((int)blockIdx.x >= tiles) {
+        adam_sweep_block(da.p + sw.lo2, da.g + sw.lo2, da.m + sw.lo2, da.v + sw.lo2, sw.n2, da.lr, da.b1, da.b2, da.eps, da.wd,
+                         da.gscale, da.step_dev, sw.vec4, sw.gate, da.halt, da.n_halt, (int)blockIdx.x - tiles,
+                         (int)gridDim.x - tiles, sc, &halted);
+        return;
+    }
+    gemm_body<32, 32, BK, 1, 1, 4, false, false, false, false, 2, true>(g, lc, smem, blockIdx.x, tiles, nullptr, &da, sc, &halted);
+}
+
 template <int BM, int BN, int BK, int KS, int PS, int WPS>
 __global__ __launch_bounds__(64 * KS, WPS) void gemm_heads_pipe_kernel(const dv_gemm_desc g, const LoadCfg lc, const dv_heads_epi he) {
     __shared__ __attribute__((aligned(1024))) float smem[gemm_smem_floats<BM, BN, BK, KS, true, true, PS>()];
@@ -1070,6 +1153,49 @@
     return gemm_launch(*d, lc, tiling, static_cast<hipStream_t>(stream));
 }
 
+extern "C" int dv_gemm_dw_adam(const dv_gemm_desc* d, float* p, const float* gr, float* m, float* v, int64_t n,
+                               const dv_adam_hyper* h, const int32_t* step_dev, int64_t lo2, int64_t hi2,
+                               const dv_wait* gate, int64_t lo, int64_t hi, const int32_t* halt, int32_t n_halt,
+                               int32_t n_sweep, dv_stream_t stream) {
+    DV_REQUIRE(d != nullptr && h != nullptr && p && gr && m && v && step_dev && n > 0);
+    DV_REQUIRE(n_halt >= 0 && (halt || n_halt == 0));
+    DV_REQUIRE(lo2 >= 0 && lo2 <= hi2 && hi2 <= n && n_sweep >= 0 && n_sweep <= 4096 && (n_sweep > 0 || lo2 == hi2));
+    DV_REQUIRE(gate == nullptr || (gate->flag && gate->ctr && gate->err && gate->max_spins > 0 && lo >= lo2 && hi >= lo &&
+                                   hi <= hi2 && n_sweep > 0));
+    LoadCfg lc;
+    int tiling = 0;
+    const int rc = gemm_prepare(d, lc, tiling);
+    if (rc != DV_OK) return rc;
+    dv_gemm_desc g = *d;
+    DV_REQUIRE(g.M > 0 && g.N > 0 && !g.a_kcontig && !g.b_kcontig && g.epilogue == DV_EPI_PLAIN && g.beta == 0.f &&
+               g.colsum_beta == 0.f && g.ldc >= g.N);
+    const int64_t c0 = g.C - gr, c1 = c0 + (int64_t)(g.M - 1) * g.ldc + g.N;
+    DV_REQUIRE(c0 >= 0 && c1 <= n && (c1 <= lo2 || c0 >= hi2 || lo2 == hi2));
+    if (g.a_colsum != nullptr) {
+        const int64_t b0 = g.a_colsum - gr, b1 = b0 + g.M;
+        DV_REQUIRE(b0 >= 0 && b1 <= n && (b1 <= lo2 || b0 >= hi2 || lo2 == hi2) && (b0 >= c1 || b1 <= c0));
+    }
+    if (tiling != 2 || !pipe_on(g) || !pipe_ok(g, lc)) return DV_ERR_UNSUPPORTED;
+    hipStream_t st = static_cast<hipStream_t>(stream);
+    {
+        const int r2 = colsum_setup(g, tiling, st);
+        if (r2 != DV_OK) return r2;
+    }
+    const int tiles32 = ((g.M + 31) / 32) * ((cols_eff(g) + 31) / 32);
+    pipe_ones_off(g);
+    const int tiles = ((g.M + 31) / 32) * ((cols_eff(g) + 31) / 32);
+    const DwAdam da{p, gr, m, v, h->lr, h->beta1, h->beta2, h->eps, h->weight_decay, h->gscale, step_dev, halt, n_halt};
+    auto al = [](const void* q) { return (reinterpret_cast<uintptr_t>(q) & 15) == 0; };
+    DwSweep sw{lo2, hi2 - lo2, al(p + lo2) && al(gr + lo2) && al(m + lo2) && al(v + lo2), AdamGate{}};
+    if (gate != nullptr) sw.gate = AdamGate{gate->flag, gate->ctr, gate->add, gate->err, gate->max_spins, lo - lo2, hi - lo2};
+    const dim3 grid((unsigned)(tiles + (hi2 > lo2 ? n_sweep : 0))), block(256);
+    if (tiles32 >= dense_min_tiles(g))
+        hipLaunchKernelGGL((gemm_dw_adam_kernel<32, DV_DENSE_WG>), grid, block, 0, st, g, lc, da, sw, tiles);
+    else
+        hipLaunchKernelGGL((gemm_dw_adam_kernel<64, 4>), grid, block, 0, st, g, lc, da, sw, tiles);
+    DV_RETURN_LAUNCH();
+}
+
 #ifdef DV_LAB
 static int heads_hb() { return 16; }
 #else
diff --git a/drvae_amd/csrc/gemm_pipe.inc b/drvae_amd/csrc/gemm_pipe.inc
--- a/drvae_amd/csrc/gemm_pipe.inc
+++ b/drvae_amd/csrc/gemm_pipe.inc
@@ -29,10 +29,14 @@
     asm volatile("s_waitcnt vmcnt(%0)" ::"n"(N) : "memory");
 }
 
+struct PipeNoFillWork {
+    __device__ __forceinline__ void operator()() const {}
+};
 template <int BM, int BN, int BK, int WM, int WN, int KS, int S, bool AKC, bool BKC, bool ONES = false, typename LineA,
-          typename LineB>
+          typename LineB, typename FillWork = PipeNoFillWork>
 __device__ __forceinline__ void pipe_loop(const dv_gemm_desc& g, float* smem, int m0, int n0, LineA a_line,
-                                          LineB b_line, f32x16 (&acc)[BM / WM / 32][BN / WN / 32]) {
+                                          LineB b_line, f32x16 (&acc)[BM / WM / 32][BN / WN / 32],
+                                          FillWork under_fill = FillWork{}) {
     using PG = PipeGeom<BM, BN, BK, WM, WN, KS, S, AKC, BKC>;
     constexpr int TM = PG::TM, TN = PG::TN, G = PG::G, P = PG::P, CPR = PG::CPR, NW = PG::NW;
     const int tid = threadIdx.x, lane = tid & 63;
@@ -179,6 +183,7 @@
         }
         issued();
     }
+    under_fill();
     asm volatile("s_waitcnt lgkmcnt(0)" ::: "memory");
     pipe_wait_vm<(S - 1) * P>();
     __builtin_amdgcn_s_barrier();
diff --git a/drvae_amd/csrc/optim.hip b/drvae_amd/csrc/optim.hip
--- a/drvae_amd/csrc/optim.hip
+++ b/drvae_amd/csrc/optim.hip
@@ -7,40 +7,7 @@
     float lr_over_bc1, inv_unused, bc2_sqrt, eps, wd, one_minus_b1, b2, one_minus_b2, gscale;
 };
 
-__device__ __forceinline__ void adam_consts(float lr, float b1, float b2, const int32_t* step_dev, float* step_size,
-                                            float* bc2_sqrt) {
-    const double t = (double)step_dev[0];
-    const double bc1 = 1.0 - pow((double)b1, t);
-    const double bc2 = 1.0 - pow((double)b2, t);
-    *step_size = (float)((double)lr / bc1);
-    *bc2_sqrt = (float)sqrt(bc2);
-}
-
-__device__ __forceinline__ void adam_one(float& p, float g, float& m, float& v, float step_size, float bc2_sqrt,
-                                         float eps, float wd, float w1, float b2, float w2, float gscale) {
-    g *= gscale;
-    if (wd != 0.f) g = g + wd * p;
-    m = m + w1 * (g - m);
-    v = v * b2 + (w2 * g) * g;
-    const float denom = sqrtf(v) / bc2_sqrt + eps;
-    p = p + (-step_size) * (m / denom);
-}
-
-__device__ __forceinline__ int any_halt(const int32_t* halt, int n_halt) {
-    int bad = 0;
-    for (int i = 0; i < n_halt; ++i)
-        bad |= __hip_atomic_load(halt + 2 * i, __ATOMIC_RELAXED, __HIP_MEMORY_SCOPE_AGENT) != 0;
-    return bad;
-}
-
-struct AdamGate {
-    int32_t* flag;
-    const int32_t* ctr;
-    int add;
-    int32_t* err;
-    int max_spins;
-    int64_t lo, hi;
-};
+#include "adam_common.inc"
 
 __global__ __launch_bounds__(256) void adam_kernel(float* __restrict__ p, const float* __restrict__ g,
                                                    float* __restrict__ m, float* __restrict__ v, int64_t n, float lr,
@@ -49,68 +16,8 @@
                                                    const int32_t* __restrict__ halt, int n_halt) {
     __shared__ float sc[2];
     __shared__ int halted;
-    bool need = false;
-    if (gate.flag != nullptr) {
-        const int64_t per = vec4 ? 4 : 1, span = (int64_t)blockDim.x * per;
-        const int64_t bstride = (int64_t)gridDim.x * span;
-        need = gate.hi > (vec4 ? ((n >> 2) << 2) : n) && gate.lo < n;
-        for (int64_t e0 = blockIdx.x * span; e0 < n; e0 += bstride) need = need || (e0 < gate.hi && e0 + span > gate.lo);
-    }
-    if (threadIdx.x == 0) {
-        int want = 0, seen = 0;
-        if (need) {
-            want = gate.ctr[0] + gate.add;
-            seen = __hip_atomic_load(gate.flag, __ATOMIC_ACQUIRE, __HIP_MEMORY_SCOPE_AGENT);
-        }
-        int h = any_halt(halt, n_halt);
-        adam_consts(lr, b1, b2, step_dev, &sc[0], &sc[1]);
-        if (need && seen - want < 0) {
-            const long long t0 = wall_clock64();
-            int k = 0;
-            while (__hip_atomic_load(gate.flag, __ATOMIC_ACQUIRE, __HIP_MEMORY_SCOPE_AGENT) - want < 0) {
-                __builtin_amdgcn_s_sleep(4);
-                if (++k > gate.max_spins) {
-                    atomicExch(gate.err, 1);
-                    break;
-                }
-            }
-            atomicAdd(gate.err + 1, (int32_t)(wall_clock64() - t0));
-            h = h || any_halt(halt, n_halt);
-        }
-        halted = h;
-    }
-    if (need) {
-        __syncthreads();
-        __builtin_amdgcn_fence(__ATOMIC_ACQUIRE, "agent");
-    }
-    __syncthreads();
-    if (halted) return;
-    const float step_size = sc[0], bc2_sqrt = sc[1];
-    const float w1 = (float)(1.0 - (double)b1), w2 = (float)(1.0 - (double)b2);
-    const int64_t stride = (int64_t)gridDim.x * blockDim.x;
-    const int64_t t0 = blockIdx.x * (int64_t)blockDim.x + threadIdx.x;
-    if (vec4) {
-        const int64_t n4 = n >> 2;
-        float4* p4 = reinterpret_cast<float4*>(p);
-        const float4* g4 = reinterpret_cast<const float4*>(g);
-        float4* m4 = reinterpret_cast<float4*>(m);
-        float4* v4 = reinterpret_cast<float4*>(v);
-        for (int64_t i = t0; i < n4; i += stride) {
-            float4 pp = p4[i], gg = g4[i], mm = m4[i], vv = v4[i];
-            adam_one(pp.x, gg.x, mm.x, vv.x, step_size, bc2_sqrt, eps, wd, w1, b2, w2, gscale);
-            adam_one(pp.y, gg.y, mm.y, vv.y, step_size, bc2_sqrt, eps, wd, w1, b2, w2, gscale);
-            adam_one(pp.z, gg.z, mm.z, vv.z, step_size, bc2_sqrt, eps, wd, w1, b2, w2, gscale);
-            adam_one(pp.w, gg.w, mm.w, vv.w, step_size, bc2_sqrt, eps, wd, w1, b2, w2, gscale);
-            p4[i] = pp;
-            m4[i] = mm;
-            v4[i] = vv;
-        }
-        for (int64_t i = (n4 << 2) + t0; i < n; i += stride)
-            adam_one(p[i], g[i], m[i], v[i], step_size, bc2_sqrt, eps, wd, w1, b2, w2, gscale);
-    } else {
-        for (int64_t i = t0; i < n; i += stride)
-            adam_one(p[i], g[i], m[i], v[i], step_size, bc2_sqrt, eps, wd, w1, b2, w2, gscale);
-    }
+    adam_sweep_block(p, g, m, v, n, lr, b1, b2, eps, wd, gscale, step_dev, vec4, gate, halt, n_halt, blockIdx.x, gridDim.x,
+                     sc, &halted);
 }
 
 typedef float adam_f4 __attribute__((ext_vector_type(4)));
diff --git a/drvae_amd/engine.py b/drvae_amd/engine.py
--- a/drvae_amd/engine.py
+++ b/drvae_amd/engine.py
@@ -654,6 +654,17 @@
                           heads.db.storage_offset() + heads.db.numel()) - g0 >= self.arena.n_live - 3)
         return ok, hs
 
+    def _fused_opt_layout(self):
+        l, g0 = self.L_enc[0], self.arena.grad.storage_offset()
+        w0, b0 = l.dW.storage_offset() - g0, l.db.storage_offset() - g0
+        end = b0 + l.db.numel()
+        ok = bool(l.g is None and not self.cfg.use_s and w0 == 0 and b0 == l.dW.shape[0] * l.dW.stride(0) and end % 4 == 0
+                  and self.cfg.optim_alg == 'adam')
+        return ok, end
+
+    def _on_device(self):
+        return self.dev.type == 'cuda'
+
     def sync_side_counters(self):
         self.side_ctr.copy_(self.step_dev)
         self.side_t.copy_(self.step_dev + 1)
@@ -818,6 +829,8 @@
                 hi = max(lc.dW.storage_offset() + span(lc.dW), lc.db.storage_offset() + lc.db.numel()) - g0
             else:
                 lo, hi = 0, 4
+                if t.fused_opt:
+                    lo, hi = t.fo_end, t.fo_end + 4
             self._adam_gate = self.sync.gate('clf_dw' if t.tail_gated else 'tail', self.step_dev, lo, hi)
             self._adam_n = t.hs if t.side_adam else None
         if t.cap_fork:
@@ -836,8 +849,20 @@
                           extra=p.DQFP if fp else None, ex_ptr=p.q_ptr if fp else None,
                           ex_rows=p.q_rows if fp else None, bump=bump, dz_add=add1,
                           prior=(p.c_klp, p.KLPraw, cfg.kl_min, Qmu) if cfg.kind == 'pvae' else None)
+        first_dw = None
+        if t.fused_opt:
+            a, gate, hs = self.arena, self._adam_gate, self._adam_n
+            assert self._ctr_bumped and len(p.enc_in) == 1 and gate is not None and hs == t.hs
+            assert t.fo_end <= gate.lo < gate.hi <= hs, 'the gated slice lies outside the sweep workgroups\' range'
+            self._adam_gate = self._adam_n = None
+            self._opt_fused = True
+
+            def first_dw(dW, dpre, x, **kw):
+                K.linear_bwd_weight_adam(dW, dpre, x, a.param, a.grad, a.exp_avg, a.exp_avg_sq, self.step_dev, lo2=t.fo_end,
+                                         hi2=hs, gate=gate, lr=cfg.learning_rate, weight_decay=cfg.weight_decay,
+                                         halt=self.sync_err, **kw)
         p.c_enc.backward(DQ, p.enc_in, None,
-                         publish_first=self.sync.pub('noise', self.step_dev, 0) if t.noise_ahead else None)
+                         publish_first=self.sync.pub('noise', self.step_dev, 0) if t.noise_ahead else None, first_dw=first_dw)
 
     def _side_backward(self, Qmu, Qlv, Z1blk, late, leaf):
         cfg, p = self.cfg, self.plan
@@ -951,6 +976,10 @@
             K.counter_add(self.step_dev, 1)
         if self._rec == 'both' and self.sched == 5 and self._dual_capable():
             K.counters_add2(self.side_ctr, 1, self.side_t, 1, publish=self.sync.pub('tail', self.side_ctr))
+        if self._opt_fused:
+            assert gscale == 1.0 and self._adam_gate is None and self._adam_n is None
+            self._opt_fused = False
+            return
         step = K.adamax_l2 if cfg.optim_alg == 'adamax' else K.adam_l2
         n = a.n_live
         if self._adam_n is not None:
diff --git a/drvae_amd/kernels.py b/drvae_amd/kernels.py
--- a/drvae_amd/kernels.py
+++ b/drvae_amd/kernels.py
@@ -824,6 +824,36 @@
                                                 _stream()), 'dv_adam_l2_gated')
 
 
+def sweep_workgroups(n):
+    return min(max((n // 4 + 255) // 256, 1), 512) if n > 0 else 0
+
+
+def dw_adam_supported(M, N, K):
+    t64, t128 = ((M + 63) // 64) * ((N + 63) // 64), ((M + 127) // 128) * ((N + 127) // 128)
+    n_fills = N * 8 >= (N + 255) // 256 * 256 * 7
+    t64_min = _TUNE.opt[3] if _TUNE.opt[3] > 0 else 1024
+    big = (t128 >= 1024 and n_fills) or (K > 256 and (t64 >= t64_min or (t64 >= 512 and K >= 8192)))
+    return bool(_TUNE.tiling == 0 and _TUNE.opt[3] != -1 and not big and M > 0 and N > 0 and K > 0)
+
+
+def linear_bwd_weight_adam(dW, dpre, x, p, g, m, v, step_dev, *, dbias=None, lo2=0, hi2=0, gate=None, n_sweep=None, lr,
+                           beta1=0.9, beta2=0.999, eps=1e-8, weight_decay=0.0, gscale=1.0, halt=None, overread=False,
+                           npad=False, publish=None):
+    assert p.is_contiguous() and g.is_contiguous() and m.is_contiguous() and v.is_contiguous()
+    assert p.numel() == g.numel() == m.numel() == v.numel()
+    d = _gemm_desc(dW, dpre, x, False, False, a_colsum=dbias, overread=overread, npad=npad, publish=publish)
+    hp, hn = _halt(halt)
+    h = _lib.AdamHyper(lr=lr, beta1=beta1, beta2=beta2, eps=eps, weight_decay=weight_decay, gscale=gscale)
+    w, lo, hi = None, 0, 0
+    if gate is not None:
+        gate = Gate(*gate)
+        w, lo, hi = _wait(Wait(gate.flag, gate.ctr, gate.err, gate.add)), gate.lo, gate.hi
+    if n_sweep is None:
+        n_sweep = sweep_workgroups(hi2 - lo2)
+    _lib.check(_lib.load().dv_gemm_dw_adam(C.byref(d), _f32(p), _f32(g), _f32(m), _f32(v), p.numel(), C.byref(h), _i32(step_dev),
+                                           lo2, hi2, w, lo, hi, hp, hn, n_sweep, _stream()), 'dv_gemm_dw_adam')
+
+
 def adamax_l2(p, g, m, u, step_dev, *, lr, beta1=0.9, beta2=0.999, eps=1e-8, weight_decay=0.0, gscale=1.0, halt=None):
     assert p.is_contiguous() and g.is_contiguous() and m.is_contiguous() and u.is_contiguous()
     hp, hn = _halt(halt)
diff --git a/drvae_amd/schedule.py b/drvae_amd/schedule.py
--- a/drvae_amd/schedule.py
+++ b/drvae_amd/schedule.py
@@ -92,6 +92,8 @@
     noise_ahead: bool = False
     klz2_on_main: bool = False
     fold_join: bool = False
+    fused_opt: bool = False
+    fo_end: int = 0
 
 _PINNED_POOL = []
 _PARTITION_STREAMS = {}
@@ -153,6 +155,7 @@
         self._ctr_bumped = False
         self._adam_n = None
         self._adam_gate = None
+        self._opt_fused = False
         self._noise_stale = True
         self._flag_side = None
         self._flags_ok = None
@@ -194,9 +197,14 @@
         tail_gated = side_adam and (p.live_feed is not None or T.get('tail_gate') == 2)
         klz2_on_main = not cfg.cont and cfg.has_y and not (p.universal and len(p.key) <= 3)
         fold_join = side_loss and cfg.has_pert and (p.B * cfg.dim_z1 + 255) // 256 <= 256
+        fo_ok, fo_end = self._fused_opt_layout()
+        fused_opt = bool(side_adam and fo_ok and fo_end + 4 <= hs and T.get('fuse_opt') and self._on_device() and
+                         K.dw_adam_supported(self.L_enc[0].N, self.L_enc[0].Kin, p.enc_in[0].shape[0]))
+        if fused_opt:
+            hs = self.arena.n_live - (self.arena.n_live - hs) * T.get('opt_split') // 3 // 4 * 4
         return Tail(dual=True, late=late, adam_gated=late and not split_kind, side_adam=side_adam, hs=hs, side_loss=side_loss,
                     cap_fork=cap_fork, tail_gated=tail_gated, noise_ahead=late or cap_fork, klz2_on_main=klz2_on_main,
-                    fold_join=fold_join)
+                    fold_join=fold_join, fused_opt=fused_opt, fo_end=fo_end if fused_opt else 0)
 
     @contextlib.contextmanager
     def _recording(self, chain, tail):
diff --git a/drvae_amd/tuning.py b/drvae_amd/tuning.py
--- a/drvae_amd/tuning.py
+++ b/drvae_amd/tuning.py
@@ -9,10 +9,13 @@
     'nll_cs': 1,
     'mmd_explicit': 1,
     'dp_fork': 1,
+    'fuse_opt': 1,
+    'opt_split': 3,
 }
 
 CHOICES = {'sched': (3, 5), 'fuse_heads': (0, 1), 'raw_heads': (1, 2), 'tail_gate': (1, 2), 'concurrent': (0, 1),
-           'nll_cs': (1, 2), 'mmd_explicit': (0, 1), 'dp_fork': (0, 1)}
+           'nll_cs': (1, 2), 'mmd_explicit': (0, 1), 'dp_fork': (0, 1), 'fuse_opt': (0, 1),
+           'opt_split': (0, 1, 2, 3)}
 
 
 def _parse():
diff --git a/include/drvae_hip.h b/include/drvae_hip.h
--- a/include/drvae_hip.h
+++ b/include/drvae_hip.h
@@ -537,6 +537,9 @@
 int dv_adam_l2_gated(float* p, const float* g, float* m, float* v, int64_t n, const dv_adam_hyper* h,
                      const int32_t* step_dev, const dv_wait* gate, int64_t lo, int64_t hi, const int32_t* halt,
                      int32_t n_halt, dv_stream_t stream);
+int dv_gemm_dw_adam(const dv_gemm_desc* d, float* p, const float* g, float* m, float* v, int64_t n,
+                    const dv_adam_hyper* h, const int32_t* step_dev, int64_t lo2, int64_t hi2, const dv_wait* gate,
+                    int64_t lo, int64_t hi, const int32_t* halt, int32_t n_halt, int32_t n_sweep, dv_stream_t stream);
 int dv_adamax_l2(float* p, const float* g, float* m, float* u, int64_t n, const dv_adam_hyper* h,
                  const int32_t* step_dev, const int32_t* halt, int32_t n_halt, dv_stream_t stream);
 int dv_counter_add(int32_t* counter_lo_hi, int32_t n_words, int64_t inc, dv_stream_t stream);
```

Measured after the change: 1.643 million samples/s, median of 2. About the same (+0.1%).
